# WildBitangent/GMU-Path-Tracer

Measured on AMD Instinct MI355X. Metric: Mpaths/s @1920x1080x64spp, 260k-tri scene, higher is better.
Workload: dtype f32; 1 GPU; config3: 259372-tri seeded sphere room (185137 nodes), 1920x1080, 64 spp steady state, UE4+glass+NEE, unbounded depth; prewarm_steps=2010, tiling=row bands x1, parallelism=tile1

## Files before the change

gmu-path-tracer_amd/build.py:

```python
import os
import subprocess
import sys

HERE = os.path.dirname(os.path.abspath(__file__))
LIB = os.path.join(HERE, "libgmupt.so")

DEVICE_SOURCES = ["csrc/pt_kernels.hip", "csrc/pt_traverse.hip", "csrc/pt_traverse_wide.hip", "csrc/pt_traverse_variants.hip", "csrc/pt_aov.hip", "csrc/pt_denoise.hip", "csrc/pt_temporal.hip", "csrc/pt_refit.hip", "csrc/pt_motion.hip", "csrc/pt_lbvh.hip", "csrc/gmupt_capi.hip"]
HOST_SOURCES = ["csrc/pt_travtables.cpp", "csrc/pt_lbvh.cpp", "host/sbvh_builder.cpp", "host/Camera.cpp", "host/TextureLoader.cpp", "host/AvirResize.cpp"]
HEADERS = ["csrc/pt_traverse_common.hpp", "csrc/pt_shading.hpp", "csrc/pt_denoise.hpp", "csrc/pt_temporal.hpp", "csrc/pt_refit.hpp", "csrc/pt_travtables.hpp", "csrc/pt_motion.hpp", "csrc/pt_lbvh.hpp", "csrc/pt_traverse_deferred.hpp", "csrc/pt_kernel_util.hpp", "host/MeshData.hpp", "host/BVHWrapper.hpp", "csrc/pt_device.hpp", "csrc/detmath.hpp", "host/sbvh_builder.hpp", "host/Camera.hpp", "host/TextureLoader.hpp", "host/png_reader.hpp", "host/Constants.hpp", "../include/gmupt.h"]

FLAGS = [
    "--offload-arch=gfx950", "-O3", "-std=c++17", "-fPIC", "-shared",
    "-ffp-contract=off", "-fhip-fp32-correctly-rounded-divide-sqrt", "-fno-gpu-flush-denormals-to-zero",
    "-fno-fast-math", "-Wall", "-Wno-unused-function",
]


TEST_BUILDS = {"variants": ["-DGMUPT_VARIANTS"], "scan1": ["-DGMUPT_SCAN_GROUP=1"],
               "wides8": ["-DGMUPT_WIDE_STACK=8", "-DGMUPT_WIDE_TOP=64", "-DGMUPT_WIDE_PARK=4"]}
EXPERIMENT_BUILDS = {"wxcd": ["-DGMUPT_WIDE_XCD_EXPERIMENT=1"], "wsg0": ["-DGMUPT_WIDE_SIGNED=0"], "mrg0": ["-DGMUPT_MATERIAL_REGROUP=0"], "wq0": ["-DGMUPT_WIDE_QUADPK=0"], "wqt0": ["-DGMUPT_WIDE_QUADTRI=0"], "dnb0": ["-DGMUPT_DN_BATCH=0"]}


def lib_path(name=None):
    return LIB if not name else os.path.join(HERE, "libgmupt_%s.so" % name)


def needs_build(name=None):
    lib = lib_path(name)
    if not os.path.exists(lib):
        return True
    t = os.path.getmtime(lib)
    deps = DEVICE_SOURCES + HOST_SOURCES + HEADERS + ["build.py"]
    return any(os.path.getmtime(os.path.join(HERE, d)) > t for d in deps if os.path.exists(os.path.join(HERE, d)))


def build(force=False, verbose=False, name=None):
    lib = lib_path(name)
    if not force and not needs_build(name):
        return lib
    hipcc = os.environ.get("HIPCC", "/opt/rocm/bin/hipcc")
    extra = os.environ.get("GMUPT_EXTRA_FLAGS", "").split() + ({**TEST_BUILDS, **EXPERIMENT_BUILDS}[name] if name else [])
    cmd = [hipcc] + FLAGS + extra + ["-x", "hip"] + [os.path.join(HERE, s) for s in DEVICE_SOURCES + HOST_SOURCES] + ["-o", lib]
    if verbose:
        print(" ".join(cmd), file=sys.stderr)
    subprocess.run(cmd, check=True, cwd=HERE)
    return lib


def build_all(force=False, verbose=False):
    from concurrent.futures import ThreadPoolExecutor
    names = [None] + sorted(TEST_BUILDS)
    with ThreadPoolExecutor(len(names)) as ex:
        return list(ex.map(lambda n: build(force=force, verbose=verbose, name=n), names))


if __name__ == "__main__":
    if "--experiments" in sys.argv:
        from concurrent.futures import ThreadPoolExecutor
        with ThreadPoolExecutor(4) as ex:
            print("\n".join(ex.map(lambda n: build(force=True, name=n), sorted(EXPERIMENT_BUILDS))))
    elif "--all" in sys.argv:
        print("\n".join(build_all(force="--force" in sys.argv, verbose=True)))
    else:
        print(build(force="--force" in sys.argv, verbose=True))
```

gmu-path-tracer_amd/capi.py:

```python
import ctypes as C
import os

import numpy as np

from . import build as _build

MAX_LIGHTS = 128
PATHCOUNT = 1 << 21
REF_GRID_THREADS = 34 * 8 * 256
STATE_BYTES = 248

(BUFFER_BVH_NODES, BUFFER_TRIANGLES, BUFFER_VERTICES, BUFFER_LIGHTS, BUFFER_TRI_PROPS, BUFFER_MATERIALS, BUFFER_TEXTURE_ARRAY) = range(7)
STAGE_SHADE, STAGE_EXTEND, STAGE_SHADOW, STAGE_RAYCASTS = range(4)
MATERIAL_UE4, MATERIAL_GLASS = 0, 1

bvh_node_dtype = np.dtype([("min", "<f4", 3), ("pad0", "<f4"), ("max", "<f4", 3), ("pad1", "<f4"),
                           ("left", "<i4"), ("right", "<i4"), ("isLeaf", "<i4"), ("pad2", "<f4")])
triangle_dtype = np.dtype([("v", "<i4", 3), ("materialID", "<u4")])
tri_props_dtype = np.dtype([("normal", "<f4", 3), ("pad0", "<f4"), ("uv", "<f4", 2), ("materialID", "<u4"), ("pad1", "<f4")])
light_dtype = np.dtype([("position", "<f4", 3), ("falloff", "<f4"), ("emission", "<f4", 3), ("radius", "<f4")])
material_dtype = np.dtype([("color", "<f4", 4), ("metallic", "<f4"), ("roughness", "<f4"), ("refractIndex", "<f4"),
                           ("transmittance", "<f4"), ("textureIndices", "<i4", 3), ("materialType", "<u4")])
assert bvh_node_dtype.itemsize == 48 and triangle_dtype.itemsize == 16 and tri_props_dtype.itemsize == 32
assert light_dtype.itemsize == 32 and material_dtype.itemsize == 48
# ... 42 lines not shown
                ("min_leaf_size", C.c_int32), ("max_leaf_size", C.c_int32), ("node_cost", C.c_float), ("tri_cost", C.c_float)]


ERR_INVALID_ARGUMENT, ERR_HIP, ERR_OUT_OF_MEMORY, ERR_NOT_BOUND, ERR_UNSUPPORTED, ERR_IO, ERR_CAST_FAULT = -1, -2, -3, -4, -5, -6, -7
MAX_TRACE_BATCH = 1 << 26


class Ray(C.Structure):
    _fields_ = [("origin", C.c_float * 3), ("tmax", C.c_float), ("direction", C.c_float * 3), ("pad", C.c_uint32)]


class Hit(C.Structure):
    _fields_ = [("t", C.c_float), ("u", C.c_float), ("v", C.c_float), ("triangle", C.c_int32), ("light", C.c_uint32),
                ("material", C.c_uint32), ("pad", C.c_uint32 * 2)]


class TraceInfo(C.Structure):
    _fields_ = [("flags", C.c_uint32), ("pad_", C.c_uint32), ("redo_rays", C.c_uint64), ("ms", C.c_double)]


class Aov(C.Structure):
    _fields_ = [("albedo", C.c_float * 3), ("depth", C.c_float), ("normal", C.c_float * 3), ("roughness", C.c_float),
                ("position", C.c_float * 3), ("metallic", C.c_float), ("triangle", C.c_int32), ("material", C.c_uint32),
                ("light", C.c_uint32), ("coverage", C.c_uint32)]


AOV_MAX_SAMPLES = 8
AOV_CHUNK_RAYS = 1 << 21
assert C.sizeof(Ray) == 32 and C.sizeof(Hit) == 32 and C.sizeof(TraceInfo) == 24 and C.sizeof(Aov) == 64
ray_dtype = np.dtype([("origin", "<f4", 3), ("tmax", "<f4"), ("direction", "<f4", 3), ("pad", "<u4")])
hit_dtype = np.dtype([("t", "<f4"), ("u", "<f4"), ("v", "<f4"), ("triangle", "<i4"), ("light", "<u4"), ("material", "<u4"), ("pad", "<u4", 2)])
aov_dtype = np.dtype([("albedo", "<f4", 3), ("depth", "<f4"), ("normal", "<f4", 3), ("roughness", "<f4"), ("position", "<f4", 3),
                      ("metallic", "<f4"), ("triangle", "<i4"), ("material", "<u4"), ("light", "<u4"), ("coverage", "<u4")])
assert ray_dtype.itemsize == 32 and hit_dtype.itemsize == 32 and aov_dtype.itemsize == 64


class DenoiseParams(C.Structure):
    _fields_ = [("passes", C.c_uint32), ("sigma_color", C.c_float), ("sigma_normal", C.c_float), ("sigma_plane", C.c_float),
                ("sigma_albedo", C.c_float)]


DENOISE_MAX_PASSES = 5
assert C.sizeof(DenoiseParams) == 20


class TemporalParams(C.Structure):
    _fields_ = [("spatial", DenoiseParams), ("history_cap", C.c_float), ("min_normal_cos", C.c_float), ("plane_dist", C.c_float)]


TEMPORAL_MAX_CAP = 65536.0
assert C.sizeof(TemporalParams) == 32
history_dtype = np.dtype([("color", "<f4", 3), ("count", "<f4"), ("normal", "<f4", 3), ("material", "<u4"), ("position", "<f4", 3),
                          ("valid", "<u4")])
assert history_dtype.itemsize == 48
motion_dtype = np.dtype([("prev_position", "<f4", 3), ("flags", "<u4")])
assert motion_dtype.itemsize == 16


class RefitInfo(C.Structure):
    _fields_ = [("rebuilt", C.c_uint32), ("reason", C.c_uint32), ("levels", C.c_uint32), ("opened_nodes", C.c_uint32), ("ms", C.c_double)]


REFIT_FLAT_CHILD, REFIT_VARIANTS_BUILD = 1, 2
assert C.sizeof(RefitInfo) == 24


class LbvhParams(C.Structure):
    _fields_ = [("max_leaf_size", C.c_uint32)]


class LbvhInfo(C.Structure):
    _fields_ = [("num_nodes", C.c_uint32), ("num_leaves", C.c_uint32), ("depth", C.c_uint32), ("num_tris", C.c_uint32),
                ("root_min", C.c_float * 3), ("root_max", C.c_float * 3), ("ms", C.c_double)]

    def as_dict(self):
        return {"num_nodes": int(self.num_nodes), "num_leaves": int(self.num_leaves), "depth": int(self.depth), "num_tris": int(self.num_tris),
                "root_min": np.array(self.root_min[:], np.float32), "root_max": np.array(self.root_max[:], np.float32), "ms": float(self.ms)}


assert C.sizeof(LbvhInfo) == 48


class GmuptError(RuntimeError):
    def __init__(self, msg, code=0):
        super().__init__(msg)
        self.code = code


_P = C.c_void_p
SYMBOLS = {
    "gmupt_device_create": (C.c_int, [C.c_int, C.POINTER(_P)]),
    "gmupt_device_destroy": (None, [_P]),
    "gmupt_last_error": (C.c_char_p, []),
    "gmupt_device_count": (C.c_int, []),
    "gmupt_buffer_create": (C.c_int, [_P, C.c_int, _P, C.c_size_t, C.POINTER(_P)]),
    "gmupt_buffer_update": (C.c_int, [_P, _P, C.c_size_t]),
    "gmupt_buffer_read": (C.c_int, [_P, _P, C.c_size_t]),
    "gmupt_buffer_destroy": (None, [_P]),
    "gmupt_buffer_size": (C.c_size_t, [_P]),
    "gmupt_texture_array_create": (C.c_int, [_P, _P, C.c_uint32, C.c_uint32, C.POINTER(_P)]),
    "gmupt_image_decode_png": (C.c_int, [_P, C.c_size_t, C.POINTER(C.c_uint32), C.POINTER(C.c_uint32), C.POINTER(_P)]),
    "gmupt_image_free": (None, [_P]),
    "gmupt_image_resize_square": (C.c_int, [_P, C.c_uint32, C.c_uint32, _P]),
    "gmupt_texture_common_size": (C.c_uint32, [C.POINTER(C.c_size_t), C.c_uint32]),
    "gmupt_renderer_create": (C.c_int, [_P, C.POINTER(RendererDesc), C.POINTER(_P)]),
    "gmupt_renderer_destroy": (None, [_P]),
    "gmupt_renderer_bind_scene": (C.c_int, [_P] * 7),
    "gmupt_renderer_bind_textures": (C.c_int, [_P, _P, _P, _P]),
    "gmupt_set_camera": (C.c_int, [_P, C.POINTER(CameraBuffer)]),
    "gmupt_iterate": (C.c_int, [_P]),
    "gmupt_resize": (C.c_int, [_P, C.c_uint32, C.c_uint32]),
    "gmupt_read_framebuffer": (C.c_int, [_P, _P, C.c_size_t]),
    "gmupt_copy_framebuffer_to_device": (C.c_int, [_P, _P, C.c_size_t]),
    "gmupt_get_counters": (C.c_int, [_P, C.POINTER(C.c_uint32 * 8)]),
    "gmupt_synchronize": (C.c_int, [_P]),
    "gmupt_get_stats": (C.c_int, [_P, C.POINTER(Stats)]),
    "gmupt_reset_stats": (C.c_int, [_P]),
    "gmupt_enable_timing": (C.c_int, [_P, C.c_int]),
    "gmupt_render_budget": (C.c_int, [_P, _P, C.c_uint32, C.POINTER(C.c_uint32)]),
    "gmupt_trace_rays": (C.c_int, [_P, _P, C.c_uint32, _P, _P, C.c_uint32, _P, C.c_uint32, C.POINTER(TraceInfo)]),
    "gmupt_camera_pick_ray": (C.c_int, [C.POINTER(CameraBuffer), C.c_float, C.c_float, C.POINTER(Ray)]),
    "gmupt_pick": (C.c_int, [_P, C.c_float, C.c_float, C.c_uint32, C.POINTER(Ray), C.POINTER(Hit)]),
    "gmupt_render_aovs": (C.c_int, [_P, C.c_uint32, _P, C.c_size_t, C.POINTER(TraceInfo)]),
    "gmupt_aov_ray": (C.c_int, [C.POINTER(CameraBuffer), C.c_uint32, C.c_uint32, C.c_uint32, C.c_uint32, C.POINTER(Ray)]),
    "gmupt_denoise_default_params": (None, [C.POINTER(DenoiseParams)]),
    "gmupt_denoise_image": (C.c_int, [_P, _P, _P, C.c_uint32, C.c_uint32, C.POINTER(DenoiseParams), _P, C.c_size_t, C.POINTER(C.c_float)]),
    "gmupt_render_denoised": (C.c_int, [_P, C.c_uint32, C.POINTER(DenoiseParams), _P, C.c_size_t, C.POINTER(TraceInfo)]),
    "gmupt_denoise_host": (C.c_int, [_P, _P, C.c_uint32, C.c_uint32, C.POINTER(DenoiseParams), _P, C.c_size_t, C.c_uint32]),
    "gmupt_temporal_default_params": (None, [C.POINTER(TemporalParams)]),
    "gmupt_temporal_create": (C.c_int, [_P, C.POINTER(_P)]),
    "gmupt_temporal_destroy": (None, [_P]),
    "gmupt_temporal_reset": (C.c_int, [_P]),
    "gmupt_temporal_denoise_image": (C.c_int, [_P, _P, _P, C.POINTER(CameraBuffer), C.c_uint32, C.c_uint32, C.c_uint32, C.c_uint32, C.c_int,
                                               C.POINTER(TemporalParams), _P, C.c_size_t, C.POINTER(C.c_float)]),
    "gmupt_render_denoised_temporal": (C.c_int, [_P, _P, C.c_uint32, C.POINTER(TemporalParams), _P, C.c_size_t, C.POINTER(TraceInfo)]),
    "gmupt_temporal_integrate_host": (C.c_int, [_P, _P, C.c_uint32, C.c_uint32, _P, C.POINTER(CameraBuffer), C.c_uint32, C.c_uint32,
                                                C.c_uint32, C.c_uint32, C.POINTER(TemporalParams), _P, _P, C.c_uint32]),
    "gmupt_bvh_refit_host": (C.c_int, [_P, C.c_uint32, _P, C.c_uint32, _P, C.c_uint32, C.c_uint32]),
    "gmupt_renderer_refit": (C.c_int, [_P, C.POINTER(RefitInfo)]),
    "gmupt_render_aovs_motion": (C.c_int, [_P, C.c_uint32, _P, C.c_uint32, _P, C.c_size_t, _P, C.c_size_t, C.POINTER(TraceInfo)]),
    "gmupt_motion_host": (C.c_int, [_P, _P, C.c_size_t, _P, C.c_uint32, _P, _P, C.c_uint32, _P]),
    "gmupt_temporal_integrate_motion_host": (C.c_int, [_P, _P, _P, C.c_uint32, C.c_uint32, _P, C.POINTER(CameraBuffer), C.c_uint32, C.c_uint32,
                                                       C.c_uint32, C.c_uint32, C.POINTER(TemporalParams), _P, _P, C.c_uint32]),
    "gmupt_temporal_denoise_image_motion": (C.c_int, [_P, _P, _P, _P, C.POINTER(CameraBuffer), C.c_uint32, C.c_uint32, C.c_uint32, C.c_uint32, C.c_int,
                                                      C.POINTER(TemporalParams), _P, C.c_size_t, C.POINTER(C.c_float)]),
    "gmupt_render_denoised_temporal_motion": (C.c_int, [_P, _P, C.c_uint32, C.POINTER(TemporalParams), _P, C.c_size_t, C.POINTER(TraceInfo)]),
    "gmupt_lbvh_default_params": (None, [C.POINTER(LbvhParams)]),
    "gmupt_lbvh_build_host": (C.c_int, [_P, C.c_uint32, _P, C.c_uint32, _P, C.POINTER(LbvhParams), _P, _P, _P, C.POINTER(LbvhInfo)]),
    "gmupt_lbvh_create": (C.c_int, [_P, C.POINTER(_P)]),
    "gmupt_lbvh_destroy": (None, [_P]),
    "gmupt_lbvh_build": (C.c_int, [_P, _P, _P, C.c_uint32, _P, C.POINTER(LbvhParams), C.POINTER(_P), C.POINTER(_P), _P, C.POINTER(LbvhInfo)]),
    "gmupt_debug_read_path_state": (C.c_int, [_P, _P, C.c_size_t]),
    "gmupt_debug_write_path_state": (C.c_int, [_P, _P, C.c_size_t]),
    "gmupt_debug_read_queues": (C.c_int, [_P, _P, C.c_size_t]),
    "gmupt_debug_write_queues": (C.c_int, [_P, _P, C.c_size_t]),
    "gmupt_debug_write_counters": (C.c_int, [_P, C.POINTER(C.c_uint32 * 8)]),
    "gmupt_debug_write_framebuffer": (C.c_int, [_P, _P, C.c_size_t]),
    "gmupt_debug_run_stage": (C.c_int, [_P, C.c_int]),
    "gmupt_debug_detmath": (C.c_int, [_P, C.c_int, _P, _P, _P, C.c_uint32]),
    "gmupt_debug_travtables_build": (C.c_int, [_P, C.c_uint32, _P, C.c_uint32, _P, C.c_uint32, C.c_int, C.c_int, C.c_int, C.POINTER(_P)]),
    "gmupt_debug_travtables_data": (_P, [_P, C.c_int, C.POINTER(C.c_size_t)]),
    "gmupt_debug_travtables_destroy": (None, [_P]),
    "gmupt_debug_wide_tables_addressable": (C.c_int, [C.c_uint32, C.c_uint32, C.c_uint32]),
    "gmupt_sbvh_default_params": (None, [C.POINTER(SbvhParams)]),
    "gmupt_sbvh_build": (C.c_int, [_P, C.c_uint32, _P, C.c_uint32, C.POINTER(SbvhParams), C.POINTER(_P)]),
    "gmupt_sbvh_num_nodes": (C.c_uint32, [_P]),
    "gmupt_sbvh_num_references": (C.c_uint32, [_P]),
    "gmupt_sbvh_sah": (C.c_float, [_P]),
    "gmupt_sbvh_depth": (C.c_uint32, [_P]),
    "gmupt_sbvh_flatten": (C.c_int, [_P, _P, _P, _P, _P]),
    "gmupt_sbvh_destroy": (None, [_P]),
    "gmupt_camera_create": (C.c_int, [C.c_uint32, C.c_uint32, C.POINTER(_P)]),
    "gmupt_camera_destroy": (None, [_P]),
    "gmupt_camera_update_resolution": (None, [_P, C.c_uint32, C.c_uint32]),
    "gmupt_camera_set_pose": (None, [_P, C.c_float, C.c_float, C.c_float, C.c_float, C.c_float]),
    "gmupt_camera_update": (None, [_P, C.c_float]),
    "gmupt_camera_set_input": (None, [_P, C.c_float, C.c_float, C.c_uint32]),
    "gmupt_camera_reset_accumulation": (None, [_P]),
    "gmupt_camera_get_buffer": (C.POINTER(CameraBuffer), [_P]),
    "gmupt_version": (C.c_char_p, []),
}

_lib = None
_libs = {}
_devices_created = 0


def _load(path):
    if path not in _libs:
        handle = C.CDLL(path)
        for name, (res, args) in SYMBOLS.items():
            fn = getattr(handle, name)
            fn.restype = res
            fn.argtypes = args
        _libs[path] = handle
    return _libs[path]


def lib():
    global _lib
    if _lib is None:
        path = os.environ.get("GMUPT_LIB") or _build.LIB
        if not os.environ.get("GMUPT_LIB") and (not os.path.exists(path) or (os.path.exists("/opt/rocm/bin/hipcc") and _build.needs_build())):
            path = _build.build()
        _lib = _load(path)
    return _lib


class use_build:

    def __init__(self, name):
        self.name = name

    def __enter__(self):
        global _lib
        path = _build.lib_path(self.name)
        if not os.path.exists(path) or (os.path.exists("/opt/rocm/bin/hipcc") and _build.needs_build(self.name)):
            if _devices_created:
                raise GmuptError("test build %r is missing or older than its sources and this process already uses the GPU: run __graft_entry__.build() first" % self.name)
            path = _build.build(name=self.name)
        self.saved = lib()
        _lib = _load(path)
        return _lib

    def __exit__(self, *exc):
        global _lib
        _lib = self.saved
        return False


def _check(rc):
    if rc != 0:
        raise GmuptError("gmupt error %d: %s" % (rc, lib().gmupt_last_error().decode(errors="replace")), rc)


def _ptr(a):
    return a.ctypes.data_as(C.c_void_p)


class Device:
    def __init__(self, index=0):
        global _devices_created
        self.h = _P()
        _check(lib().gmupt_device_create(index, C.byref(self.h)))
        _devices_created += 1
        self.index = index

    def close(self):
        if self.h:
            lib().gmupt_device_destroy(self.h)
            self.h = _P()

    def detmath(self, fn, x, y=None):
        x = np.ascontiguousarray(x, dtype=np.float32)
        y = np.zeros_like(x) if y is None else np.ascontiguousarray(y, dtype=np.float32)
        out = np.empty_like(x)
        _check(lib().gmupt_debug_detmath(self.h, fn, _ptr(x), _ptr(y), _ptr(out), x.size))
        return out


class Buffer:
    def __init__(self, dev, kind, array):
        array = np.ascontiguousarray(array)
        self.h = _P()
        self.dev = dev
        _check(lib().gmupt_buffer_create(dev.h, kind, _ptr(array), array.nbytes, C.byref(self.h)))

    @classmethod
    def wrap(cls, dev, handle):
        self = cls.__new__(cls)
        self.h, self.dev = handle, dev
        return self

    def update(self, array):
        array = np.ascontiguousarray(array)
        _check(lib().gmupt_buffer_update(self.h, _ptr(array), array.nbytes))

    def read(self, dtype=np.uint8):
        dtype = np.dtype(dtype)
        nbytes = int(lib().gmupt_buffer_size(self.h))
        out = np.empty(nbytes // dtype.itemsize, dtype=dtype)
        _check(lib().gmupt_buffer_read(self.h, _ptr(out), out.nbytes))
        return out

    def close(self):
        if self.h:
            lib().gmupt_buffer_destroy(self.h)
            self.h = _P()


class TextureArray:

    def __init__(self, dev, array):
        array = np.ascontiguousarray(array, dtype=np.uint8)
        assert array.ndim == 4 and array.shape[1] == array.shape[2] and array.shape[3] == 4
        self.h = _P()
        _check(lib().gmupt_texture_array_create(dev.h, _ptr(array), array.shape[1], array.shape[0], C.byref(self.h)))

    def close(self):
        if self.h:
            lib().gmupt_buffer_destroy(self.h)
            self.h = _P()


def decode_png(data):
    w, h, mem = C.c_uint32(), C.c_uint32(), _P()
    buf = (C.c_uint8 * len(data)).from_buffer_copy(bytes(data))
    _check(lib().gmupt_image_decode_png(buf, len(data), C.byref(w), C.byref(h), C.byref(mem)))
    try:
        out = np.ctypeslib.as_array(C.cast(mem, C.POINTER(C.c_uint8)), shape=(h.value, w.value, 4)).copy()
    finally:
        lib().gmupt_image_free(mem)
    return out


def resize_square(rgba, new_size):
    rgba = np.ascontiguousarray(rgba, dtype=np.uint8)
    assert rgba.ndim == 3 and rgba.shape[0] == rgba.shape[1] and rgba.shape[2] == 4
    out = np.empty((new_size, new_size, 4), dtype=np.uint8)
    _check(lib().gmupt_image_resize_square(_ptr(rgba), rgba.shape[0], new_size, _ptr(out)))
    return out


def texture_common_size(layer_bytes):
    arr = (C.c_size_t * len(layer_bytes))(*layer_bytes)
    return int(lib().gmupt_texture_common_size(arr, len(layer_bytes)))


def texture_array_from_png(files):
    layers = [decode_png(f) for f in files]
    for l in layers:
        if l.shape[0] != l.shape[1]:
            raise GmuptError("texture is not square")
    size = texture_common_size([l.size for l in layers])
    return np.stack([l if l.shape[0] == size else resize_square(l, size) for l in layers])


class SceneBuffers:

    def __init__(self, dev, scene):
        self.nodes = Buffer(dev, BUFFER_BVH_NODES, scene["nodes"])
        self.tris = Buffer(dev, BUFFER_TRIANGLES, scene["tris"])
        self.verts = Buffer(dev, BUFFER_VERTICES, scene["verts"])
        self.lights = Buffer(dev, BUFFER_LIGHTS, scene["lights"])
        self.props = Buffer(dev, BUFFER_TRI_PROPS, scene["props"])
        self.materials = Buffer(dev, BUFFER_MATERIALS, scene["materials"])
        self.textures = [TextureArray(dev, scene[k]) if scene.get(k) is not None else None
                         for k in ("tex_diffuse", "tex_metallic_roughness", "tex_normal")]

    def all(self):
        return [self.nodes, self.tris, self.verts, self.lights, self.props, self.materials]

    def close(self):
        for b in self.all():
            b.close()
        for t in self.textures:
            if t is not None:
                t.close()


class Camera:

    def __init__(self, width, height):
        self.h = _P()
        _check(lib().gmupt_camera_create(width, height, C.byref(self.h)))

    def set_pose(self, x, y, z, pitch, yaw):
        lib().gmupt_camera_set_pose(self.h, x, y, z, pitch, yaw)

    def update(self, dt=0.0):
        lib().gmupt_camera_update(self.h, dt)

    def update_resolution(self, width, height):
        lib().gmupt_camera_update_resolution(self.h, width, height)

    def reset_accumulation(self):
        lib().gmupt_camera_reset_accumulation(self.h)

    def set_input(self, mouse_dx=0.0, mouse_dy=0.0, w=False, s=False, a=False, d=False):
        lib().gmupt_camera_set_input(self.h, mouse_dx, mouse_dy, (1 if w else 0) | (2 if s else 0) | (4 if a else 0) | (8 if d else 0))

    @property
    def buffer(self):
        return lib().gmupt_camera_get_buffer(self.h).contents

    def buffer_copy(self):
        out = CameraBuffer()
        C.memmove(C.byref(out), C.byref(self.buffer), C.sizeof(CameraBuffer))
        return out

    def close(self):
        if self.h:
            lib().gmupt_camera_destroy(self.h)
            self.h = _P()


class Renderer:
    def __init__(self, dev, width, height, pool_paths=0, live_paths=0, tile=None, path_budget=0, max_depth=0, collect_stats=False):
        d = RendererDesc(width, height, pool_paths, live_paths, 0, 0, 0, path_budget, max_depth, 1 if collect_stats else 0)
        if tile is not None:
            d.tile_enabled, d.tile_x0, d.tile_y0 = 1, tile[0], tile[1]
        self.desc = d
        self.dev = dev
        self.h = _P()
        _check(lib().gmupt_renderer_create(dev.h, C.byref(d), C.byref(self.h)))
        self.width, self.height = width, height
        self.pool = pool_paths or PATHCOUNT
        self._scene = None
        self._temporals = []

    def bind_scene(self, sb):
        self._scene = sb
        _check(lib().gmupt_renderer_bind_scene(self.h, *[b.h for b in sb.all()]))
        _check(lib().gmupt_renderer_bind_textures(self.h, *[(t.h if t is not None else None) for t in sb.textures]))

    def refit(self):
        info = RefitInfo()
        _check(lib().gmupt_renderer_refit(self.h, C.byref(info)))
        return {k: getattr(info, k) for k, _ in RefitInfo._fields_}

    def set_camera(self, cam_buffer):
        _check(lib().gmupt_set_camera(self.h, C.byref(cam_buffer)))

    def iterate(self):
        _check(lib().gmupt_iterate(self.h))

    def run_stage(self, stage):
        _check(lib().gmupt_debug_run_stage(self.h, stage))

    def synchronize(self):
        _check(lib().gmupt_synchronize(self.h))

    def resize(self, w, h):
        _check(lib().gmupt_resize(self.h, w, h))
        self.width, self.height = w, h

    def framebuffer(self):
        out = np.empty((self.height, self.width, 4), dtype=np.float32)
        _check(lib().gmupt_read_framebuffer(self.h, _ptr(out), out.nbytes))
        return out

    def copy_framebuffer_to_device(self, device_ptr, nbytes):
        _check(lib().gmupt_copy_framebuffer_to_device(self.h, C.c_void_p(device_ptr), nbytes))

    def counters(self):
        out = (C.c_uint32 * 8)()
        _check(lib().gmupt_get_counters(self.h, C.byref(out)))
        return np.array(list(out), dtype=np.uint32)

    def stats(self, check=True):
        s = Stats()
        rc = lib().gmupt_get_stats(self.h, C.byref(s))
        if rc != ERR_CAST_FAULT or check:
            _check(rc)
        return s

    def reset_stats(self):
        _check(lib().gmupt_reset_stats(self.h))

    def enable_timing(self, mode=1):
        _check(lib().gmupt_enable_timing(self.h, int(mode)))

    def render_budget(self, camera, max_iterations=1 << 20):
        it = C.c_uint32(0)
        _check(lib().gmupt_render_budget(self.h, camera.h, max_iterations, C.byref(it)))
        return it.value

    def trace(self, closest=None, any=None, light_count=0, info=None):
        import torch
        dev = torch.device("cuda", getattr(self.dev, "index", 0))
        as_numpy = isinstance(closest, np.ndarray) or isinstance(any, np.ndarray)

        def stage(a):
            if a is None:
                return torch.empty((0, 8), dtype=torch.float32, device=dev)
            t = torch.from_numpy(np.ascontiguousarray(a, dtype=np.float32).reshape(-1, 8)).to(dev) if isinstance(a, np.ndarray) else a
            if t.dtype != torch.float32 or t.dim() != 2 or t.shape[1] != 8 or not t.is_cuda:
                raise GmuptError("trace: rays must be (N, 8) float32 on the GPU (or numpy)", ERR_INVALID_ARGUMENT)
            return t.contiguous()

        c, a = stage(closest), stage(any)
        hits = torch.empty((c.shape[0], 8), dtype=torch.float32, device=dev)
        occ = torch.empty((a.shape[0],), dtype=torch.int32, device=dev)
        torch.cuda.current_stream(dev).synchronize()
        ti = info if info is not None else TraceInfo()
        ptr = lambda t: C.c_void_p(t.data_ptr()) if t.numel() else None
        _check(lib().gmupt_trace_rays(self.h, ptr(c), c.shape[0], ptr(hits), ptr(a), a.shape[0], ptr(occ), int(light_count), C.byref(ti)))
        self.last_trace = ti
        if as_numpy:
            return hits.cpu().numpy(), occ.cpu().numpy().view(np.uint32)
        return hits, occ

    def pick(self, px, py, light_count=0):
        ray, hit = Ray(), Hit()
        _check(lib().gmupt_pick(self.h, float(px), float(py), int(light_count), C.byref(ray), C.byref(hit)))
        return ray, hit

    def aovs(self, samples=1, info=None):
        import torch
        dev = torch.device("cuda", getattr(self.dev, "index", 0))
        out = torch.empty((self.height, self.width, 16), dtype=torch.float32, device=dev)
        torch.cuda.current_stream(dev).synchronize()
        ti = info if info is not None else TraceInfo()
        _check(lib().gmupt_render_aovs(self.h, int(samples), C.c_void_p(out.data_ptr()), out.numel() * 4, C.byref(ti)))
        self.last_aovs = ti
        return out

    def aovs_motion(self, prev_verts, samples=1, info=None):
        import torch
        dev = torch.device("cuda", getattr(self.dev, "index", 0))
        if not hasattr(prev_verts, "is_cuda") or not prev_verts.is_cuda or prev_verts.dtype != torch.float32 or prev_verts.numel() % 3:
            raise GmuptError("aovs_motion: prev_verts must be a float32 tensor of 3 floats per vertex on the GPU", ERR_INVALID_ARGUMENT)
        if prev_verts.device.index != dev.index:
            raise GmuptError("aovs_motion: prev_verts lives on %s, the renderer on %s" % (prev_verts.device, dev), ERR_INVALID_ARGUMENT)
        pv = prev_verts.contiguous()
        out = torch.empty((self.height, self.width, 16), dtype=torch.float32, device=dev)
        mv = torch.empty((self.height, self.width, 4), dtype=torch.float32, device=dev)
        torch.cuda.current_stream(dev).synchronize()
        ti = info if info is not None else TraceInfo()
        _check(lib().gmupt_render_aovs_motion(self.h, int(samples), C.c_void_p(pv.data_ptr()), pv.numel() // 3, C.c_void_p(out.data_ptr()),
                                              out.numel() * 4, C.c_void_p(mv.data_ptr()), mv.numel() * 4, C.byref(ti)))
        self.last_aovs = ti
        return out, mv

    def denoise(self, aov_samples=1, info=None, **params):
        import torch
        dev = torch.device("cuda", getattr(self.dev, "index", 0))
        out = torch.empty((self.height, self.width, 4), dtype=torch.float32, device=dev)
        dp = denoise_params(**params)
        torch.cuda.current_stream(dev).synchronize()
        ti = info if info is not None else TraceInfo()
        _check(lib().gmupt_render_denoised(self.h, int(aov_samples), C.byref(dp), C.c_void_p(out.data_ptr()), out.numel() * 4, C.byref(ti)))
        self.last_denoise = ti
        return out

    def denoise_temporal(self, handle, aov_samples=1, info=None, **params):
        import torch
        dev = torch.device("cuda", getattr(self.dev, "index", 0))
        out = torch.empty((self.height, self.width, 4), dtype=torch.float32, device=dev)
        tp = temporal_params(**params)
        torch.cuda.current_stream(dev).synchronize()
        ti = info if info is not None else TraceInfo()
        _check(lib().gmupt_render_denoised_temporal(self.h, handle.h, int(aov_samples), C.byref(tp), C.c_void_p(out.data_ptr()), out.numel() * 4,
                                                    C.byref(ti)))
        self.last_denoise = ti
        return out

    def denoise_temporal_motion(self, handle, aov_samples=1, info=None, **params):
        import torch
        dev = torch.device("cuda", getattr(self.dev, "index", 0))
        out = torch.empty((self.height, self.width, 4), dtype=torch.float32, device=dev)
        tp = temporal_params(**params)
        torch.cuda.current_stream(dev).synchronize()
        ti = info if info is not None else TraceInfo()
        _check(lib().gmupt_render_denoised_temporal_motion(self.h, handle.h, int(aov_samples), C.byref(tp), C.c_void_p(out.data_ptr()),
                                                           out.numel() * 4, C.byref(ti)))
        self.last_denoise = ti
        return out

    def read_path_state(self):
        out = np.empty(self.pool * STATE_BYTES, dtype=np.uint8)
        _check(lib().gmupt_debug_read_path_state(self.h, _ptr(out), out.nbytes))
        return out

    def write_path_state(self, raw):
        raw = np.ascontiguousarray(raw, dtype=np.uint8)
        _check(lib().gmupt_debug_write_path_state(self.h, _ptr(raw), raw.nbytes))

    def read_queues(self):
        out = np.empty(self.pool * 5, dtype=np.uint32)
        _check(lib().gmupt_debug_read_queues(self.h, _ptr(out), out.nbytes))
        return out.reshape(5, self.pool)

    def write_queues(self, q):
        q = np.ascontiguousarray(q, dtype=np.uint32)
        _check(lib().gmupt_debug_write_queues(self.h, _ptr(q), q.nbytes))

    def write_counters(self, qc):
        arr = (C.c_uint32 * 8)(*[int(v) for v in qc])
        _check(lib().gmupt_debug_write_counters(self.h, C.byref(arr)))

    def write_framebuffer(self, fb):
        fb = np.ascontiguousarray(fb, dtype=np.float32)
        _check(lib().gmupt_debug_write_framebuffer(self.h, _ptr(fb), fb.nbytes))

    def close(self):
        if self.h:
            for t in self._temporals:
                t.close()
            lib().gmupt_renderer_destroy(self.h)
            self.h = _P()


class Temporal:

    def __init__(self, renderer):
        self.renderer = renderer
        self.h = _P()
        _check(lib().gmupt_temporal_create(renderer.h, C.byref(self.h)))
        renderer._temporals.append(self)

    def reset(self):
        _check(lib().gmupt_temporal_reset(self.h))

    def close(self):
        if self.h:
            lib().gmupt_temporal_destroy(self.h)
            self.h = _P()


def camera_pick_ray(cam_buffer, px, py):
    ray = Ray()
    _check(lib().gmupt_camera_pick_ray(C.byref(cam_buffer), float(px), float(py), C.byref(ray)))
    return ray


def hit_fields(hits):
    h = hits.cpu().numpy() if hasattr(hits, "cpu") else np.asarray(hits)
    rec = np.ascontiguousarray(h, dtype=np.float32).reshape(-1, 8).view(hit_dtype)[:, 0]
    return {k: rec[k].copy() for k in ("t", "u", "v", "triangle", "light", "material")}


def aov_ray(cam_buffer, x, y, samples, k):
    ray = Ray()
    _check(lib().gmupt_aov_ray(C.byref(cam_buffer), int(x), int(y), int(samples), int(k), C.byref(ray)))
    return ray


def aov_rays(cam_buffer, xs, ys, samples):
    R = 1 if samples == 1 else samples * samples + 1
    out = np.empty((len(xs), R, 8), np.float32)
    for i, (x, y) in enumerate(zip(xs, ys)):
        for k in range(R):
            out[i, k] = np.frombuffer(bytes(aov_ray(cam_buffer, x, y, samples, k)), np.float32)
    return out


def aov_fields(aovs):
    a = aovs.cpu().numpy() if hasattr(aovs, "cpu") else np.asarray(aovs)
    a = np.ascontiguousarray(a, dtype=np.float32)
    rec = a.reshape(-1, 16).view(aov_dtype)[:, 0]
    shape = a.shape[:-1]
    return {k: rec[k].reshape(shape + rec[k].shape[1:]).copy() for k in aov_dtype.names}


def denoise_params(**params):
    dp = DenoiseParams()
    lib().gmupt_denoise_default_params(C.byref(dp))
    for k, v in params.items():
        if k not in ("passes", "sigma_color", "sigma_normal", "sigma_plane", "sigma_albedo"):
            raise TypeError("unknown denoiser parameter %r" % k)
        setattr(dp, k, v)
    return dp


def denoise_image(renderer, beauty, aov, ms=None, **params):
    import torch
    if beauty.dim() != 3 or beauty.shape[2] != 4 or aov.dim() != 3 or aov.shape[2] != 16 or tuple(aov.shape[:2]) != tuple(beauty.shape[:2]):
        raise GmuptError("denoise_image: beauty must be (H, W, 4) and aov (H, W, 16)", ERR_INVALID_ARGUMENT)
    if beauty.dtype != torch.float32 or aov.dtype != torch.float32 or not beauty.is_cuda or not aov.is_cuda:
        raise GmuptError("denoise_image: float32 tensors on the GPU", ERR_INVALID_ARGUMENT)
    beauty, aov = beauty.contiguous(), aov.contiguous()
    H, W = beauty.shape[0], beauty.shape[1]
    out = torch.empty_like(beauty)
    dp = denoise_params(**params)
    torch.cuda.current_stream(beauty.device).synchronize()
    t = C.c_float(0.0)
    _check(lib().gmupt_denoise_image(renderer.h, C.c_void_p(beauty.data_ptr()), C.c_void_p(aov.data_ptr()), W, H, C.byref(dp),
                                     C.c_void_p(out.data_ptr()), out.numel() * 4, C.byref(t)))
    if ms is not None:
        ms.append(t.value)
    return out


def denoise_host(beauty, aov, threads=16, **params):
    b = beauty.cpu().numpy() if hasattr(beauty, "cpu") else np.asarray(beauty)
    a = aov.cpu().numpy() if hasattr(aov, "cpu") else np.asarray(aov)
    b = np.ascontiguousarray(b, dtype=np.float32)
    if a.dtype == aov_dtype:
        a = a.view(np.float32).reshape(a.shape + (16,))
    a = np.ascontiguousarray(a, dtype=np.float32)
    if b.ndim != 3 or b.shape[2] != 4 or a.shape != b.shape[:2] + (16,):
        raise GmuptError("denoise_host: beauty must be (H, W, 4) and aov (H, W, 16)", ERR_INVALID_ARGUMENT)
    out = np.empty_like(b)
    dp = denoise_params(**params)
    _check(lib().gmupt_denoise_host(_ptr(b), _ptr(a), b.shape[1], b.shape[0], C.byref(dp), _ptr(out), out.nbytes, int(threads)))
    return out


TEMPORAL_FIELDS = ("history_cap", "min_normal_cos", "plane_dist")


def temporal_params(**params):
    tp = TemporalParams()
    lib().gmupt_temporal_default_params(C.byref(tp))
    for k, v in params.items():
        if k in TEMPORAL_FIELDS:
            setattr(tp, k, v)
        elif k in ("passes", "sigma_color", "sigma_normal", "sigma_plane", "sigma_albedo"):
            setattr(tp.spatial, k, v)
        else:
            raise TypeError("unknown temporal denoiser parameter %r" % k)
    return tp


def temporal_denoise_image(handle, beauty, aov, cam_buffer, new_accumulation, origin=(0, 0), ms=None, motion=None, **params):
    import torch
    if beauty.dim() != 3 or beauty.shape[2] != 4 or aov.dim() != 3 or aov.shape[2] != 16 or tuple(aov.shape[:2]) != tuple(beauty.shape[:2]):
        raise GmuptError("temporal_denoise_image: beauty must be (H, W, 4) and aov (H, W, 16)", ERR_INVALID_ARGUMENT)
    if beauty.dtype != torch.float32 or aov.dtype != torch.float32 or not beauty.is_cuda or not aov.is_cuda:
        raise GmuptError("temporal_denoise_image: float32 tensors on the GPU", ERR_INVALID_ARGUMENT)
    beauty, aov = beauty.contiguous(), aov.contiguous()
    H, W = beauty.shape[0], beauty.shape[1]
    out = torch.empty_like(beauty)
    tp = temporal_params(**params)
    if motion is not None:
        if motion.dtype != torch.float32 or not motion.is_cuda or tuple(motion.shape) != (H, W, 4) or motion.device != beauty.device:
            raise GmuptError("temporal_denoise_image: motion must be an (H, W, 4) float32 tensor on the GPU of beauty", ERR_INVALID_ARGUMENT)
        hdev = getattr(handle.renderer.dev, "index", 0)
        if beauty.device.index != hdev or aov.device != beauty.device:
# ... 247 lines not shown
```

gmu-path-tracer_amd/csrc/gmupt_capi.hip:

```cpp
#include "pt_device.hpp"
#include "detmath.hpp"
#include "pt_shading.hpp"
#include "pt_denoise.hpp"
#include "pt_temporal.hpp"
#include "pt_refit.hpp"
#include "pt_motion.hpp"
#include "pt_travtables.hpp"
#include "pt_lbvh.hpp"
#include "../host/sbvh_builder.hpp"
#include "../host/Camera.hpp"
#include "../host/TextureLoader.hpp"
#include "../host/png_reader.hpp"

#include <hip/hip_runtime.h>
#include <algorithm>
#include <array>
#include <cmath>
#include <cstdarg>
#include <cstdio>
#include <cstdlib>
#include <cstring>
#include <limits>
#include <string>
#include <unordered_map>
// ... 167 lines not shown
extern "C" uint32_t gmupt_texture_common_size(const size_t* layer_bytes, uint32_t layers)
{
    if (!layer_bytes || layers == 0) return 0;
    return gmupt::commonDimension(std::vector<size_t>(layer_bytes, layer_bytes + layers));
}

extern "C" int gmupt_texture_array_create(gmupt_device* dev, const uint8_t* rgba8, uint32_t size, uint32_t layers, gmupt_buffer** out)
{
    if (!dev || !out || !rgba8) return fail(GMUPT_ERR_INVALID_ARGUMENT, "gmupt_texture_array_create: null argument");
    if (size == 0 || layers == 0 || size > 16384) return fail(GMUPT_ERR_INVALID_ARGUMENT, "gmupt_texture_array_create: %u layers of %ux%u", layers, size, size);
    int rc = gmupt_buffer_create(dev, GMUPT_BUFFER_TEXTURE_ARRAY, rgba8, (size_t)size * size * layers * 4, out);
    if (rc == GMUPT_OK) { (*out)->texSize = size; (*out)->texLayers = layers; }
    return rc;
}

extern "C" int gmupt_buffer_update(gmupt_buffer* buf, const void* data, size_t bytes)
{
    if (!buf || (!data && bytes)) return fail(GMUPT_ERR_INVALID_ARGUMENT, "gmupt_buffer_update: null argument");
    if (bytes > buf->bytes) return fail(GMUPT_ERR_INVALID_ARGUMENT, "gmupt_buffer_update: %zu bytes into a %zu-byte buffer", bytes, buf->bytes);
    HIP_TRY(hipSetDevice(buf->dev->id));
    HIP_TRY(hipDeviceSynchronize());
    HIP_TRY(hipMemcpy(buf->dptr, data, bytes, hipMemcpyHostToDevice));
    return GMUPT_OK;
}

extern "C" int gmupt_buffer_read(const gmupt_buffer* buf, void* dst, size_t bytes)
{
    if (!buf || (!dst && bytes)) return fail(GMUPT_ERR_INVALID_ARGUMENT, "gmupt_buffer_read: null argument");
    if (bytes > buf->bytes) return fail(GMUPT_ERR_INVALID_ARGUMENT, "gmupt_buffer_read: %zu bytes from a %zu-byte buffer", bytes, buf->bytes);
    HIP_TRY(hipSetDevice(buf->dev->id));
    HIP_TRY(hipDeviceSynchronize());
    HIP_TRY(hipMemcpy(dst, buf->dptr, bytes, hipMemcpyDeviceToHost));
    return GMUPT_OK;
}

extern "C" void gmupt_buffer_destroy(gmupt_buffer* buf)
{
    if (!buf) return;
    (void)hipSetDevice(buf->dev->id);
    (void)hipFree(buf->dptr);
    delete buf;
}

extern "C" size_t gmupt_buffer_size(const gmupt_buffer* buf) { return buf ? buf->bytes : 0; }

struct StageEvents { hipEvent_t e[5]; bool extOnly = false; };

struct gmupt_renderer {
    gmupt_device* dev = nullptr;
    gmupt_renderer_desc desc{};
    hipStream_t stream = nullptr;
    RenderParams p{};
    bool sceneBound = false, cameraSet = false;
    uint64_t iterations = 0;
    uint32_t travBlocks = 0;
    int timing = 0;
    std::vector<StageEvents> evPool; size_t evUsed = 0;
    double msStage[4] = { 0, 0, 0, 0 }; uint64_t timedIters = 0;
    std::vector<void*> allocs;
    void* travNodes = nullptr; void* travTris = nullptr; void* travRecs = nullptr; void* travWide = nullptr; void* travPairs = nullptr; void* travPairRef = nullptr;
    int travMode = 70;
    uint32_t castFlags = 0;
    uint32_t* queryCounters = nullptr; DevStats* queryStats = nullptr; void* pickBuf = nullptr;
    hipEvent_t queryEv[2] = { nullptr, nullptr };
    gmupt_ray* aovRays = nullptr; gmupt_hit* aovHits = nullptr;
    void* dnScratch = nullptr; size_t dnScratchBytes = 0;
    void* dnInput = nullptr; size_t dnInputBytes = 0;
    hipEvent_t dnEv[2] = { nullptr, nullptr };
    uint64_t accumGeneration = 0;
    uint64_t bindingId = 0, geomGeneration = 0;
    const gmupt_buffer* boundNodes = nullptr; const gmupt_buffer* boundTris = nullptr; const gmupt_buffer* boundVerts = nullptr;
    size_t boundElems[3] = { 0, 0, 0 };
    std::vector<uint32_t> rfLevelNodes, rfLevelOff, rfNodeMap, rfWideMap, rfOpened;
    void* rfDev = nullptr;
    hipEvent_t rfEv[2] = { nullptr, nullptr };
};

static std::array<void**, 6> trav_tables(gmupt_renderer* r) { return { &r->travNodes, &r->travTris, &r->travRecs, &r->travWide, &r->travPairs, &r->travPairRef }; }

static int dev_alloc(gmupt_renderer* r, void** ptr, size_t bytes, int fill)
{
    *ptr = nullptr;
    HIP_TRY(hipMalloc(ptr, bytes ? bytes : 16));
    r->allocs.push_back(*ptr);
    HIP_TRY(hipMemsetAsync(*ptr, fill, bytes ? bytes : 16, r->stream));
    return GMUPT_OK;
}

static int alloc_framebuffer(gmupt_renderer* r, uint32_t w, uint32_t h)
{
    void* fb = nullptr; void* head = nullptr;
    const size_t npix = (size_t)w * h;
    HIP_TRY(hipMalloc(&fb, npix * 16 + 16));
    HIP_TRY(hipMalloc(&head, npix * 4 + 16));
    HIP_TRY(hipMemsetAsync(fb, 0, npix * 16 + 16, r->stream));
    HIP_TRY(hipMemsetAsync(head, 0xFF, npix * 4 + 16, r->stream));
    r->p.fb = (float4*)fb; r->p.listHead = (uint32_t*)head; r->p.fbW = w; r->p.fbH = h;
    return GMUPT_OK;
}

extern "C" void gmupt_renderer_destroy(gmupt_renderer* r)
{
    if (!r) return;
    (void)hipSetDevice(r->dev->id);
    if (r->stream) (void)hipStreamSynchronize(r->stream);
    for (auto& se : r->evPool) for (auto& e : se.e) (void)hipEventDestroy(e);
    for (hipEvent_t e : r->queryEv) if (e) (void)hipEventDestroy(e);
    for (hipEvent_t e : r->dnEv) if (e) (void)hipEventDestroy(e);
    for (hipEvent_t e : r->rfEv) if (e) (void)hipEventDestroy(e);
    if (r->rfDev) (void)hipFree(r->rfDev);
    for (void* a : r->allocs) (void)hipFree(a);
    if (r->dnScratch) (void)hipFree(r->dnScratch);
    if (r->dnInput) (void)hipFree(r->dnInput);
    if (r->p.fb) (void)hipFree(r->p.fb);
    if (r->p.listHead) (void)hipFree(r->p.listHead);
    for (void** t : trav_tables(r)) if (*t) (void)hipFree(*t);
    if (r->stream) (void)hipStreamDestroy(r->stream);
    delete r;
}

static int parse_traversal_mode(const char* tv)
{
    constexpr int kDefault = 70;
    if (!tv || !*tv) return kDefault;
    if (std::strcmp(tv, "whilewhile") == 0) return 0;
    if (std::strcmp(tv, "ref") == 0) return 1;
    if (std::strcmp(tv, "static") == 0) return 2;
    if (std::strncmp(tv, "ifif", 4) == 0) return 3 + std::atoi(tv + 4);
    if (std::strcmp(tv, "coop") == 0) return 20;
    if (std::strcmp(tv, "top") == 0) return 30;
    if (std::strncmp(tv, "def", 3) == 0) return 40 + std::atoi(tv + 3);
    if (std::strncmp(tv, "pipe", 4) == 0) return 50 + std::atoi(tv + 4);
    if (std::strncmp(tv, "cast", 4) == 0) return 60 + std::atoi(tv + 4);
    if (std::strcmp(tv, "wide") == 0) return 70;
    return kDefault;
}

extern "C" int gmupt_renderer_create(gmupt_device* dev, const gmupt_renderer_desc* desc, gmupt_renderer** out)
{
    if (!dev || !desc || !out) return fail(GMUPT_ERR_INVALID_ARGUMENT, "gmupt_renderer_create: null argument");
    *out = nullptr;
    if (desc->width == 0 || desc->height == 0) return fail(GMUPT_ERR_INVALID_ARGUMENT, "gmupt_renderer_create: empty accumulation target %ux%u", desc->width, desc->height);
    gmupt_renderer* r = new (std::nothrow) gmupt_renderer();
    if (!r) return fail(GMUPT_ERR_OUT_OF_MEMORY, "gmupt_renderer_create: out of host memory");
    r->dev = dev; r->desc = *desc;
    r->travMode = parse_traversal_mode(std::getenv("GMUPT_TRAVERSAL"));
    if (!traversal_mode_available(r->travMode)) {
        delete r;
        return fail(GMUPT_ERR_UNSUPPORTED, "gmupt_renderer_create: GMUPT_TRAVERSAL=%s is not part of this build (wide, cast0 and def0 are; the other rungs need -DGMUPT_VARIANTS)", std::getenv("GMUPT_TRAVERSAL"));
    }
    if (r->desc.pool_paths == 0) r->desc.pool_paths = GMUPT_PATHCOUNT;
    if (r->desc.live_paths == 0 || r->desc.live_paths > r->desc.pool_paths) r->desc.live_paths = r->desc.pool_paths;
    const uint32_t P = r->desc.pool_paths, L = r->desc.live_paths;
    if ((uint64_t)P * F_COUNT * 4ull > (200ull << 30)) { delete r; return fail(GMUPT_ERR_INVALID_ARGUMENT, "gmupt_renderer_create: pool of %u paths is too large", P); }

    hipError_t e = hipSetDevice(dev->id);
    if (e == hipSuccess) e = hipStreamCreateWithFlags(&r->stream, hipStreamNonBlocking);
    if (e != hipSuccess) { delete r; return fail(GMUPT_ERR_HIP, "gmupt_renderer_create: %s", hipGetErrorString(e)); }

    RenderParams& p = r->p;
    p.P = P; p.L = L;
    p.nBlocks = (L + kBlock - 1) / kBlock;
    p.tileEnabled = desc->tile_enabled; p.tileX0 = desc->tile_x0; p.tileY0 = desc->tile_y0;
    p.budget = desc->path_budget; p.maxDepth = desc->max_depth;
    const uint32_t tb = traversal_block_threads();
    r->travBlocks = (L + tb - 1) / tb;
    p.ovfStride = r->travBlocks * tb;
    if (p.ovfStride < deferred_block_threads()) p.ovfStride = deferred_block_threads();
    { const char* rw = std::getenv("GMUPT_RAYS_PER_WAVE"); p.raysPerWave = rw ? (uint32_t)std::atoi(rw) : 128u; if (p.raysPerWave < 64) p.raysPerWave = 64; if (r->travMode >= 60 && p.raysPerWave > 128) p.raysPerWave = 128;  }
    { const char* wpc = std::getenv("GMUPT_WAVES_PER_CU"); const uint32_t w = wpc ? (uint32_t)std::atoi(wpc) : 16u; const uint32_t db = deferred_block_threads(); p.travGridBlocks = (uint32_t)dev->prop.multiProcessorCount * ((w * 64 + db - 1) / db); if (p.travGridBlocks * db > p.ovfStride) p.travGridBlocks = p.ovfStride / db; if (p.travGridBlocks == 0) p.travGridBlocks = 1; }
    { const char* ep = std::getenv("GMUPT_EXTEND_PRUNE"); p.extendPrune = ep ? (uint32_t)std::atoi(ep) : 0u; }
    { const char* sp = std::getenv("GMUPT_SHADOW_PRUNE"); p.shadowPrune = sp ? (uint32_t)std::atoi(sp) : 0u; }
    { const char* ws = std::getenv("GMUPT_WIDE_STEPS"); p.tuneWideSteps = ws ? (uint32_t)std::atoi(ws) : 0u; }
    { const char* xb = std::getenv("GMUPT_XCD_BINS"); p.xcdBins = xb ? (uint32_t)std::atoi(xb) : 0u; }
    { const char* lc = std::getenv("GMUPT_CAST_LOOP_CAP"); p.castLoopCap = lc ? (uint32_t)std::atoi(lc) : (1u << 20); if (p.castLoopCap == 0) p.castLoopCap = 1u << 20; }
    { const char* e1 = std::getenv("GMUPT_REFILL"); p.tuneRefill = e1 ? (uint32_t)std::atoi(e1) : 20u; const char* e2 = std::getenv("GMUPT_TRI_THRESH"); p.tuneTriThresh = e2 ? (uint32_t)std::atoi(e2) : ((r->travMode == 60 || r->travMode == 63 || r->travMode == 70) ? 24u : 32u); }

    int rc = GMUPT_OK;
    { const char* pad = std::getenv("GMUPT_STATE_PAD"); p.PS = P + (pad ? (uint32_t)std::atoi(pad) & ~63u : 1088u); }
    if (rc == GMUPT_OK) rc = dev_alloc(r, (void**)&p.state, (size_t)F_COUNT * p.PS * 4, 0);
    if (rc == GMUPT_OK) rc = dev_alloc(r, (void**)&p.cls, (size_t)P, CLS_ENDED);
    if (rc == GMUPT_OK) rc = dev_alloc(r, (void**)&p.listNext, (size_t)P * 4, 0xFF);
    if (rc == GMUPT_OK) rc = dev_alloc(r, (void**)&p.sample, (size_t)P * 12, 0);
    if (rc == GMUPT_OK) rc = dev_alloc(r, (void**)&p.blockCounts, (size_t)p.nBlocks * 4 * kNumCounts, 0);
    p.nGroups = (p.nBlocks + kScanGroup - 1) / kScanGroup; p.groupParity = 0;
    if (rc == GMUPT_OK) rc = dev_alloc(r, (void**)&p.groupTotals, (size_t)2 * kNumCounts * p.nGroups * 4, 0);
    if (rc == GMUPT_OK) rc = dev_alloc(r, (void**)&p.queues, (size_t)P * 20, 0);
    if (rc == GMUPT_OK) rc = dev_alloc(r, (void**)&p.qc, 32, 0);
    if (rc == GMUPT_OK) rc = dev_alloc(r, (void**)&p.stats, sizeof(DevStats), 0);
    if (rc == GMUPT_OK) rc = dev_alloc(r, (void**)&p.travCounters, 128, 0);
    if (rc == GMUPT_OK) rc = dev_alloc(r, (void**)&p.ovfStack, (size_t)p.ovfStride * traversal_overflow_entries() * 4, 0);
    if (rc == GMUPT_OK) rc = alloc_framebuffer(r, desc->width, desc->height);
    if (rc == GMUPT_OK) {
        DevStats init{}; init.activePaths = L;
        e = hipMemcpyAsync(p.stats, &init, sizeof(init), hipMemcpyHostToDevice, r->stream);
        if (e == hipSuccess) e = hipStreamSynchronize(r->stream);
        if (e != hipSuccess) rc = fail(GMUPT_ERR_HIP, "gmupt_renderer_create: %s", hipGetErrorString(e));
    }
    if (rc != GMUPT_OK) { std::string keep = g_lastError; gmupt_renderer_destroy(r); g_lastError = keep; return rc; }
    *out = r;
    return GMUPT_OK;
}

static TravOptions trav_options(bool wantWide)
{
    const char* order = std::getenv("GMUPT_TOP_ORDER");
    const char* pairing = std::getenv("GMUPT_NODE_PAIRING");
    TravOptions o;
    o.wantWide = wantWide; o.topOrderBfs = order && std::strcmp(order, "bfs") == 0; o.nodePairing = !(pairing && std::atoi(pairing) == 0);
    o.topCapacity = traversal_top_capacity; o.wideTopCapacity = traversal_wide_top_capacity();
    return o;
}

static int build_traversal_copy(gmupt_renderer* r, const gmupt_buffer* nodesB, const gmupt_buffer* trisB, const gmupt_buffer* vertsB)
{
    HIP_TRY(hipSetDevice(r->dev->id));
    HIP_TRY(hipStreamSynchronize(r->stream));
    const size_t N = nodesB->elems, R = trisB->elems, V = vertsB->elems;
    std::vector<gmupt_bvh_node> nodes(N);
    std::vector<gmupt_triangle> tris(R ? R : 1);
    std::vector<float> verts(V ? V * 3 : 3);
    HIP_TRY(hipMemcpy(nodes.data(), nodesB->dptr, N * sizeof(gmupt_bvh_node), hipMemcpyDeviceToHost));
    if (R) HIP_TRY(hipMemcpy(tris.data(), trisB->dptr, R * sizeof(gmupt_triangle), hipMemcpyDeviceToHost));
    if (V) HIP_TRY(hipMemcpy(verts.data(), vertsB->dptr, V * 12, hipMemcpyDeviceToHost));

    TravTables tt;
    const std::string err = build_trav_tables(nodes.data(), N, tris.data(), R, verts.data(), V, trav_options(r->travMode == 70), tt);
    if (!err.empty()) return fail(GMUPT_ERR_INVALID_ARGUMENT, "%s", err.c_str());

    const bool haveWide = !tt.wide.empty();
    const void* recs = nullptr; size_t recBytes = 0;
#ifdef GMUPT_VARIANTS
    recs = tt.recs.data(); recBytes = tt.recs.size() * sizeof(Rec64);
#endif
    const struct { const void* data; size_t bytes; } up[6] = {
        { tt.nodes.data(), tt.nodes.size() * sizeof(Node64) }, { tt.tris.data(), tt.tris.size() * sizeof(Tri48) }, { recs, recBytes },
        { tt.wide.data(), tt.wide.size() * sizeof(WNode) }, { tt.pairs.data(), haveWide ? tt.pairs.size() * sizeof(TriPair) : 0 },
        { tt.pairRef.data(), haveWide ? tt.pairRef.size() * 4 : 0 } };
    const std::array<void**, 6> dst = trav_tables(r);
    for (int k = 0; k < 6; k++) {
        if (*dst[k]) { HIP_TRY(hipFree(*dst[k])); *dst[k] = nullptr; }
        if (!up[k].bytes) continue;
        HIP_TRY(hipMalloc(dst[k], up[k].bytes));
        HIP_TRY(hipMemcpy(*dst[k], up[k].data, up[k].bytes, hipMemcpyHostToDevice));
    }
    TravScene& t = r->p.trav;
    t.recs = (const Rec64*)r->travRecs; t.nodes = (const Node64*)r->travNodes; t.tris = (const Tri48*)r->travTris;
    t.wnodes = (const WNode*)r->travWide; t.pairs = (const TriPair*)r->travPairs; t.pairRef = (const uint32_t*)r->travPairRef;
    t.triBase = tt.s.triBase; t.rootDesc = tt.s.rootDesc; t.topCount = tt.s.topCount; t.topCountDeep = tt.s.topCountDeep; t.maxDepth = tt.s.maxDepth;
    for (int k = 0; k < 3; k++) { t.rootMin[k] = tt.s.rootMin[k]; t.rootMax[k] = tt.s.rootMax[k]; }
    t.wideCount = tt.s.wideCount; t.wideTopCount = tt.s.wideTopCount; t.wideStackBound = tt.s.wideStackBound; t.wideRootDesc = 0; t.numPairs = tt.s.numPairs;

    if (r->rfDev) { HIP_TRY(hipFree(r->rfDev)); r->rfDev = nullptr; }
    r->rfLevelNodes.swap(tt.levelNodes); r->rfLevelOff.swap(tt.levelOff); r->rfNodeMap.swap(tt.nodeMap); r->rfWideMap.swap(tt.wideMap); r->rfOpened.swap(tt.opened);
    r->boundNodes = nodesB; r->boundTris = trisB; r->boundVerts = vertsB;
    r->boundElems[0] = N; r->boundElems[1] = R; r->boundElems[2] = V;
    return GMUPT_OK;
}

static_assert(sizeof(gmupt_refit_info) == 24 && offsetof(gmupt_refit_info, ms) == 16, "gmupt_refit_info layout");

extern "C" int gmupt_renderer_refit(gmupt_renderer* r, gmupt_refit_info* info)
{
    if (!r) return fail(GMUPT_ERR_INVALID_ARGUMENT, "gmupt_renderer_refit: null renderer");
    if (info) *info = gmupt_refit_info{};
    if (!r->sceneBound) return fail(GMUPT_ERR_NOT_BOUND, "gmupt_renderer_refit: no scene bound");
    if (r->boundNodes->elems != r->boundElems[0] || r->boundTris->elems != r->boundElems[1] || r->boundVerts->elems != r->boundElems[2])
        return fail(GMUPT_ERR_INVALID_ARGUMENT, "gmupt_renderer_refit: the bound buffers hold (%zu, %zu, %zu) nodes / triangle records / vertices, at bind time (%zu, %zu, %zu)",
                    r->boundNodes->elems, r->boundTris->elems, r->boundVerts->elems, r->boundElems[0], r->boundElems[1], r->boundElems[2]);
    HIP_TRY(hipSetDevice(r->dev->id));
    HIP_TRY(hipStreamSynchronize(r->stream));
    const std::vector<uint32_t>* maps[4] = { &r->rfLevelNodes, &r->rfNodeMap, &r->rfWideMap, &r->rfOpened };
    size_t off[4], words = 16;
    for (int k = 0; k < 4; k++) { off[k] = words; words += (maps[k]->size() + 3) & ~(size_t)3; }
    if (!r->rfDev) {
        HIP_TRY(hipMalloc(&r->rfDev, words * 4));
        for (int k = 0; k < 4; k++)
            if (!maps[k]->empty()) HIP_TRY(hipMemcpy((uint32_t*)r->rfDev + off[k], maps[k]->data(), maps[k]->size() * 4, hipMemcpyHostToDevice));
    }
    for (hipEvent_t& e : r->rfEv) if (!e) HIP_TRY(hipEventCreate(&e));
    uint32_t* dev = (uint32_t*)r->rfDev;
    const TravScene& t = r->p.trav;
    RfArgs a{};
    a.nodes = (DNode*)r->boundNodes->dptr; a.tris = (const gmupt_triangle*)r->boundTris->dptr; a.verts = (const float*)r->boundVerts->dptr;
    a.numNodes = (uint32_t)r->boundElems[0]; a.numTris = (uint32_t)r->boundElems[1]; a.numVerts = (uint32_t)r->boundElems[2];
    a.levelNodes = dev + off[0];
    a.ttris = (Tri48*)r->travTris; a.pairs = (TriPair*)r->travPairs; a.pairRef = t.pairRef; a.numPairs = t.numPairs;
    a.tnodes = (Node64*)r->travNodes; a.nodeMap = dev + off[1]; a.numPacked = (uint32_t)r->rfNodeMap.size();
    a.wnodes = (WNode*)r->travWide; a.wideMap = dev + off[2]; a.wideCount = r->travWide ? t.wideCount : 0u;
    a.opened = dev + off[3]; a.numOpened = r->travWide ? (uint32_t)r->rfOpened.size() : 0u;
    a.flags = dev;

    uint32_t back[16] = { 0 };
    HIP_TRY(hipMemsetAsync(dev, 0, 64, r->stream));
    launch_refit_check(a, r->stream);
    HIP_TRY(hipGetLastError());
    HIP_TRY(hipMemcpyAsync(back, dev, 4, hipMemcpyDeviceToHost, r->stream));
    HIP_TRY(hipStreamSynchronize(r->stream));
    if (back[0] & kRfFlagBadIndex) return fail(GMUPT_ERR_INVALID_ARGUMENT, "gmupt_renderer_refit: a triangle record references a vertex outside the vertex buffer (the triangle records changed since bind)");
    if (back[0] & kRfFlagNonFinite) return fail(GMUPT_ERR_INVALID_ARGUMENT, "gmupt_renderer_refit: a vertex used by a triangle record is not finite; nothing was written");

    uint32_t reason = 0;
#ifdef GMUPT_VARIANTS
    reason = GMUPT_REFIT_VARIANTS_BUILD;
#endif
    HIP_TRY(hipEventRecord(r->rfEv[0], r->stream));
    const uint32_t levels = launch_refit_boxes(a, r->rfLevelOff, r->stream);
    if (!reason) launch_refit_tables(a, r->stream);
    HIP_TRY(hipGetLastError());
    HIP_TRY(hipMemcpyAsync(dev + 4, a.nodes, 32, hipMemcpyDeviceToDevice, r->stream));
    HIP_TRY(hipEventRecord(r->rfEv[1], r->stream));
    HIP_TRY(hipMemcpyAsync(back, dev, 64, hipMemcpyDeviceToHost, r->stream));
    HIP_TRY(hipStreamSynchronize(r->stream));
    float ms = 0.0f;
    HIP_TRY(hipEventElapsedTime(&ms, r->rfEv[0], r->rfEv[1]));
    if (back[1]) reason |= GMUPT_REFIT_FLAT_CHILD;
    const uint32_t openedNodes = a.numOpened;
    if (reason) {
        int rc = build_traversal_copy(r, r->boundNodes, r->boundTris, r->boundVerts);
        if (rc != GMUPT_OK) return rc;
    } else {
        for (int k = 0; k < 3; k++) { std::memcpy(&r->p.trav.rootMin[k], &back[4 + k], 4); std::memcpy(&r->p.trav.rootMax[k], &back[8 + k], 4); }
    }
    r->geomGeneration++;
    if (info) { info->rebuilt = reason ? 1u : 0u; info->reason = reason; info->levels = levels; info->opened_nodes = openedNodes; info->ms = (double)ms; }
    return GMUPT_OK;
}

extern "C" int gmupt_bvh_refit_host(gmupt_bvh_node* nodes, uint32_t num_nodes, const gmupt_triangle* tris, uint32_t num_tris,
                                    const float* verts, uint32_t num_verts, uint32_t threads)
{
    if (!nodes || num_nodes == 0 || (!tris && num_tris) || (!verts && num_verts)) return fail(GMUPT_ERR_INVALID_ARGUMENT, "gmupt_bvh_refit_host: null or empty array");
    const std::string err = validate_tree("gmupt_bvh_refit_host", nodes, num_nodes, tris, num_tris, num_verts, 0);
// ... 783 lines not shown
    if (rc != GMUPT_OK) return rc;
    HIP_TRY(hipSetDevice(r->dev->id));
    const bool fold = !t->seen || t->generation != r->accumGeneration;
    TpSlot& fz = fold ? t->last : t->frozen;
    TpSlot& nw = fold ? t->frozen : t->last;
    const uint32_t nv = r->p.scene.numVerts;
    const auto inPose = [&](const TpSlot& sl) { return sl.hasPose && sl.binding == r->bindingId && sl.numVerts == nv; };
    const bool moved = poses && fz.present && inPose(fz) && fz.geomGeneration != r->geomGeneration;
    const size_t npix = (size_t)W * H;
    rc = grow_scratch(r, &r->dnInput, &r->dnInputBytes, npix * (sizeof(gmupt_aov) + 16 + (moved ? sizeof(gmupt_motion) : 0)));
    if (rc != GMUPT_OK) return rc;
    gmupt_aov* aov = static_cast<gmupt_aov*>(r->dnInput);
    float* beauty = reinterpret_cast<float*>(static_cast<char*>(r->dnInput) + npix * sizeof(gmupt_aov));
    gmupt_motion* motion = moved ? reinterpret_cast<gmupt_motion*>(static_cast<char*>(r->dnInput) + npix * (sizeof(gmupt_aov) + 16)) : nullptr;
    gmupt_trace_info ai;
    if (moved) rc = gmupt_render_aovs_motion(r, aov_samples, static_cast<const float*>(fz.verts), nv, aov, npix * sizeof(gmupt_aov), motion, npix * sizeof(gmupt_motion), &ai);
    else rc = gmupt_render_aovs(r, aov_samples, aov, npix * sizeof(gmupt_aov), &ai);
    if (info) *info = ai;
    if (rc != GMUPT_OK) return rc;
    rc = gmupt_copy_framebuffer_to_device(r, beauty, npix * 16);
    if (rc != GMUPT_OK) return rc;
    if (poses && !(inPose(nw) && nw.geomGeneration == r->geomGeneration)) {
        nw.hasPose = false;
        rc = grow_scratch(r, &nw.verts, &nw.vertsBytes, (size_t)nv * 12);
        if (rc != GMUPT_OK) return rc;
        HIP_TRY(hipMemcpyAsync(nw.verts, r->p.scene.verts, (size_t)nv * 12, hipMemcpyDeviceToDevice, r->stream));
    }
    const uint32_t x0 = r->p.tileEnabled ? r->p.tileX0 : 0u, y0 = r->p.tileEnabled ? r->p.tileY0 : 0u;
    float ms = 0.0f;
    rc = temporal_denoise(fn, t, beauty, aov, motion, &r->p.cam, x0, y0, W, H, fold ? 1 : 0, p, out_rgba, bytes, &ms);
    if (info) info->ms = ai.ms + ms;
    if (rc != GMUPT_OK) return rc;
    t->seen = true; t->generation = r->accumGeneration;
    if (poses) { t->last.hasPose = true; t->last.binding = r->bindingId; t->last.geomGeneration = r->geomGeneration; t->last.numVerts = nv; }
    return GMUPT_OK;
}

static int temporal_integrate_host(const char* fn, const float* beauty_rgba, const gmupt_aov* aov, const gmupt_motion* motion, uint32_t width, uint32_t height,
                                   const gmupt_history* prev, const gmupt_camera_buffer* prev_cam, uint32_t prev_x0, uint32_t prev_y0,
                                   uint32_t prev_width, uint32_t prev_height, const gmupt_temporal_params* p,
                                   float* out_rgba, gmupt_history* out_history, uint32_t threads)
{
    if (!beauty_rgba || !aov || !out_rgba || !out_history) return fail(GMUPT_ERR_INVALID_ARGUMENT, "%s: null beauty, aov or output", fn);
    if (width == 0 || height == 0 || width > 65535 || height > 65535 || (uint64_t)width * height > (1ull << 28))
        return fail(GMUPT_ERR_INVALID_ARGUMENT, "%s: image of %ux%u (1..65535 each, at most 2^28 pixels)", fn, width, height);
    if (prev) {
        if (!prev_cam) return fail(GMUPT_ERR_INVALID_ARGUMENT, "%s: a previous record set without its camera", fn);
        if (prev_width == 0 || prev_height == 0 || prev_width > 65535 || prev_height > 65535 || (uint64_t)prev_width * prev_height > (1ull << 28) ||
            prev_x0 > 65535 || prev_y0 > 65535)
            return fail(GMUPT_ERR_INVALID_ARGUMENT, "%s: previous rectangle of %ux%u at (%u, %u) (1..65535 each, at most 2^28 pixels)", fn, prev_width, prev_height, prev_x0, prev_y0);
    }
    {
        const size_t n = (size_t)width * height;
        const uintptr_t o[2] = { (uintptr_t)out_rgba, (uintptr_t)out_history }, on[2] = { n * 16, n * sizeof(gmupt_history) };
        const uintptr_t i[5] = { (uintptr_t)beauty_rgba, (uintptr_t)aov, (uintptr_t)prev, (uintptr_t)motion, (uintptr_t)out_history },
                        in[5] = { n * 16, n * sizeof(gmupt_aov), prev ? (size_t)prev_width * prev_height * sizeof(gmupt_history) : 0,
                                  motion ? n * sizeof(gmupt_motion) : 0, n * sizeof(gmupt_history) };
        for (int a = 0; a < 2; a++)
            for (int b = 0; b < (a == 0 ? 5 : 4); b++)
                if (in[b] && o[a] < i[b] + in[b] && i[b] < o[a] + on[a]) return fail(GMUPT_ERR_INVALID_ARGUMENT, "%s: an output overlaps another array", fn);
    }
    gmupt_temporal_params d;
    if (!p) { gmupt_temporal_default_params(&d); p = &d; }
    DnParams dn; TpParams tp;
    int rc = temporal_params(fn, p, dn, tp);
    if (rc != GMUPT_OK) return rc;
    try {
        temporal_host(beauty_rgba, aov, motion, (int)width, (int)height, prev, prev_cam, (int)prev_x0, (int)prev_y0, (int)prev_width, (int)prev_height, tp,
                      out_rgba, out_history, (int)std::min(std::max(threads, 1u), 16u));
    } catch (const std::bad_alloc&) {
        return fail(GMUPT_ERR_OUT_OF_MEMORY, "%s: out of host memory for %ux%u pixels", fn, width, height);
    } catch (const std::exception& e) {
        return fail(GMUPT_ERR_INVALID_ARGUMENT, "%s: %s", fn, e.what());
    }
    return GMUPT_OK;
}

extern "C" int gmupt_temporal_integrate_host(const float* beauty_rgba, const gmupt_aov* aov, uint32_t width, uint32_t height,
                                             const gmupt_history* prev, const gmupt_camera_buffer* prev_cam, uint32_t prev_x0, uint32_t prev_y0,
                                             uint32_t prev_width, uint32_t prev_height, const gmupt_temporal_params* p,
                                             float* out_rgba, gmupt_history* out_history, uint32_t threads)
{
    return temporal_integrate_host("gmupt_temporal_integrate_host", beauty_rgba, aov, nullptr, width, height, prev, prev_cam, prev_x0, prev_y0, prev_width,
                                   prev_height, p, out_rgba, out_history, threads);
}

extern "C" int gmupt_temporal_integrate_motion_host(const float* beauty_rgba, const gmupt_aov* aov, const gmupt_motion* motion, uint32_t width, uint32_t height,
                                                    const gmupt_history* prev, const gmupt_camera_buffer* prev_cam, uint32_t prev_x0, uint32_t prev_y0,
                                                    uint32_t prev_width, uint32_t prev_height, const gmupt_temporal_params* p,
                                                    float* out_rgba, gmupt_history* out_history, uint32_t threads)
{
    return temporal_integrate_host("gmupt_temporal_integrate_motion_host", beauty_rgba, aov, motion, width, height, prev, prev_cam, prev_x0, prev_y0, prev_width,
                                   prev_height, p, out_rgba, out_history, threads);
}

extern "C" int gmupt_motion_host(const gmupt_hit* hits, const gmupt_aov* aov, size_t n, const gmupt_triangle* tris, uint32_t num_tris,
                                 const float* verts_now, const float* verts_prev, uint32_t num_verts, gmupt_motion* out)
{
    const char* fn = "gmupt_motion_host";
    if (n == 0) return GMUPT_OK;
    if (!hits || !aov || !out || !tris || !verts_now || !verts_prev) return fail(GMUPT_ERR_INVALID_ARGUMENT, "%s: null array", fn);
    for (size_t i = 0; i < n; i++) {
        gmupt_hit h;
        std::memcpy(&h, (const char*)hits + i * sizeof(h), sizeof(h));
        if (h.triangle < 0 || h.light > 0u) continue;
        if ((uint32_t)h.triangle >= num_tris) return fail(GMUPT_ERR_INVALID_ARGUMENT, "%s: hit %zu names triangle record %d of %u", fn, i, h.triangle, num_tris);
        gmupt_triangle T;
        std::memcpy(&T, (const char*)tris + (size_t)h.triangle * sizeof(T), sizeof(T));
        for (int k = 0; k < 3; k++)
            if (T.v[k] < 0 || (uint32_t)T.v[k] >= num_verts) return fail(GMUPT_ERR_INVALID_ARGUMENT, "%s: triangle record %d references vertex %d of %u", fn, h.triangle, T.v[k], num_verts);
    }
    motion_host(hits, aov, n, tris, verts_now, verts_prev, out);
    return GMUPT_OK;
}

struct gmupt_camera { Camera cam; gmupt_camera(uint32_t w, uint32_t h) : cam(w, h) {} };

extern "C" int gmupt_render_budget(gmupt_renderer* r, gmupt_camera* cam, uint32_t max_iterations, uint32_t* iters)
{
    if (!r || !cam) return fail(GMUPT_ERR_INVALID_ARGUMENT, "gmupt_render_budget: null argument");
    if (!r->desc.path_budget) return fail(GMUPT_ERR_INVALID_ARGUMENT, "gmupt_render_budget: renderer was created without a path_budget");
    HIP_TRY(hipSetDevice(r->dev->id));
    static_assert(offsetof(DevStats, stackOverflow) == offsetof(DevStats, activePaths) + 4, "the drain check reads both words with one copy");
    uint32_t* hostActive = nullptr;
    HIP_TRY(hipHostMalloc((void**)&hostActive, 8, hipHostMallocDefault));
    hostActive[0] = 1; hostActive[1] = 0;
    uint32_t k = 0;
    int rc = GMUPT_OK;
    constexpr uint32_t kDrainHorizon = 512;
    uint32_t drainStart = 0xFFFFFFFFu;
    for (; k < max_iterations; k++) {
        cam->cam.update(0.0f);
        rc = gmupt_set_camera(r, cam->cam.getBuffer());
        if (rc == GMUPT_OK) rc = gmupt_iterate(r);
        if (rc != GMUPT_OK) break;
        if ((k & 7u) == 7u) {
            hipError_t e = hipMemcpyAsync(hostActive, &r->p.stats->activePaths, 8, hipMemcpyDeviceToHost, r->stream);
            if (e == hipSuccess) e = hipStreamSynchronize(r->stream);
            if (e != hipSuccess) { rc = fail(GMUPT_ERR_HIP, "gmupt_render_budget: %s", hipGetErrorString(e)); break; }
            if (hostActive[1] & 3u) { rc = fail(GMUPT_ERR_CAST_FAULT, "gmupt_render_budget: a ray-cast launch flagged its results as invalid after %u iterations (flags %#x)", k + 1, hostActive[1]); k++; break; }
            if (*hostActive == 0) { k++; break; }
            if (*hostActive < r->p.L && drainStart == 0xFFFFFFFFu) drainStart = k;
            if (drainStart != 0xFFFFFFFFu && k - drainStart >= kDrainHorizon) { k++; break; }
        }
    }
    (void)hipHostFree(hostActive);
    if (rc == GMUPT_OK) { hipError_t e = hipStreamSynchronize(r->stream); if (e != hipSuccess) rc = fail(GMUPT_ERR_HIP, "gmupt_render_budget: %s", hipGetErrorString(e)); }
    if (rc == GMUPT_OK) rc = check_cast_flags(r, "gmupt_render_budget");
    if (iters) *iters = k;
    return rc;
}

namespace {
struct FieldMap { uint32_t refOffset, slotBytes, comps, first; };
const FieldMap kFieldMap[] = {
    { 0, 16, 3, F_RAY_OX }, { 16, 16, 3, F_RAY_DX }, { 32, 16, 3, F_MAT_R }, { 48, 8, 2, F_MAT_METALLIC }, { 56, 16, 3, F_NRM_X },
    { 72, 16, 3, F_SP_X }, { 88, 16, 3, F_BARY_X }, { 104, 4, 1, F_HIT_DIST }, { 108, 16, 4, F_TRI_0 }, { 124, 16, 3, F_SH_OX },
    { 140, 16, 3, F_SH_DX }, { 156, 4, 1, F_LIGHT_IDX }, { 160, 4, 1, F_LIGHT_DIST }, { 164, 4, 1, F_IN_SHADOW }, { 168, 16, 3, F_RAD_R },
    { 184, 16, 3, F_THR_R }, { 200, 16, 3, F_LTHR_R }, { 216, 16, 3, F_DL_R }, { 232, 4, 1, F_PATH_LEN }, { 236, 8, 2, F_SCR_X }, { 244, 4, 1, F_IS_EMITTER },
};
}

extern "C" int gmupt_debug_read_path_state(gmupt_renderer* r, void* dst, size_t bytes)
{
    if (!r || !dst) return fail(GMUPT_ERR_INVALID_ARGUMENT, "gmupt_debug_read_path_state: null argument");
    const size_t P = r->p.P;
    if (bytes < P * GMUPT_STATE_BYTES) return fail(GMUPT_ERR_INVALID_ARGUMENT, "gmupt_debug_read_path_state: %zu bytes given, %zu needed", bytes, P * (size_t)GMUPT_STATE_BYTES);
    HIP_TRY(hipSetDevice(r->dev->id));
    const size_t PS = r->p.PS;
    std::vector<uint32_t> soa((size_t)F_COUNT * PS);
    HIP_TRY(hipMemcpyAsync(soa.data(), r->p.state, soa.size() * 4, hipMemcpyDeviceToHost, r->stream));
    HIP_TRY(hipStreamSynchronize(r->stream));
    std::memset(dst, 0, P * GMUPT_STATE_BYTES);
    uint8_t* out = (uint8_t*)dst;
    for (const FieldMap& f : kFieldMap)
        for (size_t i = 0; i < P; i++) {
            uint32_t* o = (uint32_t*)(out + (size_t)f.refOffset * P + (size_t)f.slotBytes * i);
            for (uint32_t c = 0; c < f.comps; c++) o[c] = soa[(size_t)(f.first + c) * PS + i];
        }
    return GMUPT_OK;
}

extern "C" int gmupt_debug_write_path_state(gmupt_renderer* r, const void* src, size_t bytes)
{
    if (!r || !src) return fail(GMUPT_ERR_INVALID_ARGUMENT, "gmupt_debug_write_path_state: null argument");
    const size_t P = r->p.P;
    if (bytes < P * GMUPT_STATE_BYTES) return fail(GMUPT_ERR_INVALID_ARGUMENT, "gmupt_debug_write_path_state: %zu bytes given, %zu needed", bytes, P * (size_t)GMUPT_STATE_BYTES);
    HIP_TRY(hipSetDevice(r->dev->id));
    const size_t PS = r->p.PS;
    std::vector<uint32_t> soa((size_t)F_COUNT * PS);
    const uint8_t* in = (const uint8_t*)src;
    for (const FieldMap& f : kFieldMap)
        for (size_t i = 0; i < P; i++) {
            const uint32_t* o = (const uint32_t*)(in + (size_t)f.refOffset * P + (size_t)f.slotBytes * i);
            for (uint32_t c = 0; c < f.comps; c++) soa[(size_t)(f.first + c) * PS + i] = o[c];
        }
    HIP_TRY(hipMemcpyAsync(r->p.state, soa.data(), soa.size() * 4, hipMemcpyHostToDevice, r->stream));
    HIP_TRY(hipStreamSynchronize(r->stream));
    return GMUPT_OK;
}

extern "C" int gmupt_debug_read_queues(gmupt_renderer* r, uint32_t* dst, size_t bytes)
{
    if (!r || !dst) return fail(GMUPT_ERR_INVALID_ARGUMENT, "gmupt_debug_read_queues: null argument");
    const size_t need = (size_t)r->p.P * 20;
    if (bytes < need) return fail(GMUPT_ERR_INVALID_ARGUMENT, "gmupt_debug_read_queues: %zu bytes given, %zu needed", bytes, need);
    HIP_TRY(hipSetDevice(r->dev->id));
    HIP_TRY(hipMemcpyAsync(dst, r->p.queues, need, hipMemcpyDeviceToHost, r->stream));
    HIP_TRY(hipStreamSynchronize(r->stream));
    return GMUPT_OK;
}

extern "C" int gmupt_debug_write_queues(gmupt_renderer* r, const uint32_t* src, size_t bytes)
{
    if (!r || !src) return fail(GMUPT_ERR_INVALID_ARGUMENT, "gmupt_debug_write_queues: null argument");
    const size_t need = (size_t)r->p.P * 20;
    if (bytes < need) return fail(GMUPT_ERR_INVALID_ARGUMENT, "gmupt_debug_write_queues: %zu bytes given, %zu needed", bytes, need);
    HIP_TRY(hipSetDevice(r->dev->id));
    HIP_TRY(hipMemcpyAsync(r->p.queues, src, need, hipMemcpyHostToDevice, r->stream));
    HIP_TRY(hipStreamSynchronize(r->stream));
    return GMUPT_OK;
}

extern "C" int gmupt_debug_write_counters(gmupt_renderer* r, const uint32_t in[8])
{
    if (!r || !in) return fail(GMUPT_ERR_INVALID_ARGUMENT, "gmupt_debug_write_counters: null argument");
    HIP_TRY(hipSetDevice(r->dev->id));
    HIP_TRY(hipMemcpyAsync(r->p.qc, in, 32, hipMemcpyHostToDevice, r->stream));
    HIP_TRY(hipStreamSynchronize(r->stream));
    return GMUPT_OK;
}

extern "C" int gmupt_debug_write_framebuffer(gmupt_renderer* r, const float* rgba, size_t bytes)
{
    if (!r || !rgba) return fail(GMUPT_ERR_INVALID_ARGUMENT, "gmupt_debug_write_framebuffer: null argument");
    const size_t need = (size_t)r->p.fbW * r->p.fbH * 16;
    if (bytes < need) return fail(GMUPT_ERR_INVALID_ARGUMENT, "gmupt_debug_write_framebuffer: %zu bytes given, %zu needed", bytes, need);
    HIP_TRY(hipSetDevice(r->dev->id));
    HIP_TRY(hipMemcpyAsync(r->p.fb, rgba, need, hipMemcpyHostToDevice, r->stream));
    HIP_TRY(hipStreamSynchronize(r->stream));
    return GMUPT_OK;
}

extern "C" int gmupt_debug_detmath(gmupt_device* dev, int fn, const float* x, const float* y, float* out, uint32_t n)
{
    if (!dev || !x || !y || !out) return fail(GMUPT_ERR_INVALID_ARGUMENT, "gmupt_debug_detmath: null argument");
    if (n == 0) return GMUPT_OK;
    HIP_TRY(hipSetDevice(dev->id));
    float *dx = nullptr, *dy = nullptr, *dout = nullptr;
    HIP_TRY(hipMalloc((void**)&dx, (size_t)n * 4)); HIP_TRY(hipMalloc((void**)&dy, (size_t)n * 4)); HIP_TRY(hipMalloc((void**)&dout, (size_t)n * 4));
    HIP_TRY(hipMemcpy(dx, x, (size_t)n * 4, hipMemcpyHostToDevice)); HIP_TRY(hipMemcpy(dy, y, (size_t)n * 4, hipMemcpyHostToDevice));
    launch_detmath(fn, dx, dy, dout, n, nullptr);
    HIP_TRY(hipGetLastError());
    HIP_TRY(hipMemcpy(out, dout, (size_t)n * 4, hipMemcpyDeviceToHost));
    (void)hipFree(dx); (void)hipFree(dy); (void)hipFree(dout);
    return GMUPT_OK;
}

static_assert(sizeof(gmupt_lbvh_info) == 48 && offsetof(gmupt_lbvh_info, ms) == 40, "gmupt_lbvh_info layout");

extern "C" void gmupt_lbvh_default_params(gmupt_lbvh_params* p) { if (p) p->max_leaf_size = 4; }

static void lbvh_fill_info(gmupt_lbvh_info* info, const LbResult& res, uint32_t numTris, double ms)
{
    if (!info) return;
    info->num_nodes = res.numNodes; info->num_leaves = res.numLeaves; info->depth = res.depth; info->num_tris = numTris;
    for (int k = 0; k < 3; k++) { info->root_min[k] = res.rootMin[k]; info->root_max[k] = res.rootMax[k]; }
    info->ms = ms;
}

static int lbvh_leaf_size(const char* fn, const gmupt_lbvh_params* params, uint32_t* L)
{
    *L = params ? params->max_leaf_size : 4u;
    if (*L < 1 || *L > kLbMaxLeaf) return fail(GMUPT_ERR_INVALID_ARGUMENT, "%s: max_leaf_size %u outside 1..%u", fn, *L, kLbMaxLeaf);
    return GMUPT_OK;
}

extern "C" int gmupt_lbvh_build_host(const float* verts, uint32_t num_verts, const int32_t* indices, uint32_t num_tris, const uint32_t* vertex_material,
                                     const gmupt_lbvh_params* params, gmupt_bvh_node* nodes_out, gmupt_triangle* tris_out, int32_t* ref_triangle_out,
                                     gmupt_lbvh_info* info)
{
    if (!verts || !indices || !nodes_out || !tris_out || num_verts == 0 || num_tris == 0) return fail(GMUPT_ERR_INVALID_ARGUMENT, "gmupt_lbvh_build_host: null or empty array");
    if (num_tris > kLbMaxTris) return fail(GMUPT_ERR_INVALID_ARGUMENT, "gmupt_lbvh_build_host: more than 2^30 triangles");
    uint32_t L;
    int rc = lbvh_leaf_size("gmupt_lbvh_build_host", params, &L);
    if (rc != GMUPT_OK) return rc;
    LbResult res{};
    int status = GMUPT_OK;
    const std::string err = lbvh_build_host(verts, num_verts, indices, num_tris, vertex_material, L, nodes_out, tris_out, ref_triangle_out, res, &status);
    if (status != GMUPT_OK) return fail(status, "gmupt_lbvh_build_host: %s", err.c_str());
    lbvh_fill_info(info, res, num_tris, 0.0);
    return GMUPT_OK;
}

struct gmupt_lbvh { gmupt_device* dev; hipStream_t stream = nullptr; hipEvent_t ev[2] = { nullptr, nullptr }; void* scratch = nullptr; uint32_t capTris = 0; size_t sortTemp = 0; };

extern "C" int gmupt_lbvh_create(gmupt_device* dev, gmupt_lbvh** out)
{
    if (!dev || !out) return fail(GMUPT_ERR_INVALID_ARGUMENT, "gmupt_lbvh_create: null argument");
    *out = nullptr;
    gmupt_lbvh* h = new (std::nothrow) gmupt_lbvh();
    if (!h) return fail(GMUPT_ERR_OUT_OF_MEMORY, "gmupt_lbvh_create: out of host memory");
    h->dev = dev;
    hipError_t e = hipSetDevice(dev->id);
    if (e == hipSuccess) e = hipStreamCreate(&h->stream);
    for (hipEvent_t& ev : h->ev) if (e == hipSuccess) e = hipEventCreate(&ev);
    if (e != hipSuccess) { gmupt_lbvh_destroy(h); return fail(GMUPT_ERR_HIP, "gmupt_lbvh_create: %s", hipGetErrorString(e)); }
    *out = h;
    return GMUPT_OK;
}

extern "C" void gmupt_lbvh_destroy(gmupt_lbvh* h)
{
    if (!h) return;
    (void)hipSetDevice(h->dev->id);
    if (h->stream) { (void)hipStreamSynchronize(h->stream); (void)hipStreamDestroy(h->stream); }
    for (hipEvent_t ev : h->ev) if (ev) (void)hipEventDestroy(ev);
    if (h->scratch) (void)hipFree(h->scratch);
    delete h;
}

static int lbvh_output_buffer(gmupt_device* dev, gmupt_buffer_kind kind, size_t elems, const void* src, hipStream_t s, gmupt_buffer** out)
{
    gmupt_buffer* b = new (std::nothrow) gmupt_buffer();
    if (!b) return fail(GMUPT_ERR_OUT_OF_MEMORY, "gmupt_lbvh_build: out of host memory");
    b->dev = dev; b->kind = kind; b->elems = elems; b->bytes = elems * kind_stride(kind); b->dptr = nullptr;
    hipError_t e = hipMalloc(&b->dptr, b->bytes + 16);
    if (e == hipSuccess) e = hipMemsetAsync((char*)b->dptr + b->bytes, 0, 16, s);
    if (e == hipSuccess) e = hipMemcpyAsync(b->dptr, src, b->bytes, hipMemcpyDeviceToDevice, s);
    if (e != hipSuccess) { if (b->dptr) (void)hipFree(b->dptr); delete b; return fail(GMUPT_ERR_HIP, "gmupt_lbvh_build(%zu bytes): %s", elems * kind_stride(kind), hipGetErrorString(e)); }
    *out = b;
    return GMUPT_OK;
}

extern "C" int gmupt_lbvh_build(gmupt_lbvh* h, const gmupt_buffer* vertices, const int32_t* device_indices, uint32_t num_tris, const uint32_t* device_vertex_material,
                                const gmupt_lbvh_params* params, gmupt_buffer** nodes_out, gmupt_buffer** triangles_out, int32_t* device_ref_triangle,
                                gmupt_lbvh_info* info)
{
    if (nodes_out) *nodes_out = nullptr;
    if (triangles_out) *triangles_out = nullptr;
    if (!h || !vertices || !device_indices || !nodes_out || !triangles_out) return fail(GMUPT_ERR_INVALID_ARGUMENT, "gmupt_lbvh_build: null argument");
    if (vertices->kind != GMUPT_BUFFER_VERTICES || vertices->dev != h->dev) return fail(GMUPT_ERR_INVALID_ARGUMENT, "gmupt_lbvh_build: not a vertex buffer of the builder's device");
    if (vertices->elems == 0 || num_tris == 0) return fail(GMUPT_ERR_INVALID_ARGUMENT, "gmupt_lbvh_build: empty mesh");
    if (num_tris > kLbMaxTris || vertices->elems > 0x7FFFFFFFu) return fail(GMUPT_ERR_INVALID_ARGUMENT, "gmupt_lbvh_build: more than 2^30 triangles or 2^31 - 1 vertices");
    if (((uintptr_t)device_indices | (uintptr_t)device_vertex_material | (uintptr_t)device_ref_triangle) & 3) return fail(GMUPT_ERR_INVALID_ARGUMENT, "gmupt_lbvh_build: misaligned pointer");
    uint32_t L;
    int rc = lbvh_leaf_size("gmupt_lbvh_build", params, &L);
    if (rc != GMUPT_OK) return rc;
    HIP_TRY(hipSetDevice(h->dev->id));
    size_t sortTemp = 0;
    HIP_TRY(lbvh_sort_temp_bytes(num_tris, &sortTemp));
// ... 97 lines not shown
```

gmu-path-tracer_amd/csrc/pt_device.hpp:

```cpp
#pragma once
#include <hip/hip_runtime.h>
#include <cstdint>
#include "../../include/gmupt.h"

namespace gmupt {

enum Field : uint32_t {
    F_RAY_OX, F_RAY_OY, F_RAY_OZ, F_RAY_DX, F_RAY_DY, F_RAY_DZ,
    F_MAT_R, F_MAT_G, F_MAT_B, F_MAT_METALLIC, F_MAT_ROUGHNESS,
    F_NRM_X, F_NRM_Y, F_NRM_Z,
    F_SP_X, F_SP_Y, F_SP_Z,
    F_BARY_X, F_BARY_Y, F_BARY_Z,
    F_HIT_DIST,
    F_TRI_0, F_TRI_1, F_TRI_2, F_TRI_MAT,
    F_SH_OX, F_SH_OY, F_SH_OZ, F_SH_DX, F_SH_DY, F_SH_DZ,
    F_LIGHT_IDX, F_LIGHT_DIST, F_IN_SHADOW,
    F_RAD_R, F_RAD_G, F_RAD_B,
    F_THR_R, F_THR_G, F_THR_B,
    F_LTHR_R, F_LTHR_G, F_LTHR_B,
    F_DL_R, F_DL_G, F_DL_B,
    F_PATH_LEN, F_SCR_X, F_SCR_Y, F_IS_EMITTER,
    F_COUNT
};
static_assert(F_COUNT == 50, "50 words per path");

enum SlotClass : uint8_t { CLS_UE4 = 0, CLS_GLASS = 1, CLS_ENDED = 2, CLS_RETIRED = 3, CLS_NONE = 4, CLS_MASK = 0x0F, CLS_SHADOW_BIT = 0x10 };
constexpr int kNumCounts = 4;
#ifndef GMUPT_SCAN_GROUP
#define GMUPT_SCAN_GROUP 64
#endif
constexpr uint32_t kScanGroup = GMUPT_SCAN_GROUP;

enum Counter : uint32_t { QC_NEWPATH = 0, QC_LASTPATHCNT = 1, QC_MATUE4 = 2, QC_MATGLASS = 3, QC_EXT_UE4_OFFSET = 4, QC_EXT_GLASS_OFFSET = 5, QC_SHADOWRAY = 6, QC_EXT_COUNT = 7 };
enum Queue : uint32_t { Q_NEWPATH = 0, Q_MAT_UE4 = 1, Q_MAT_GLASS = 2, Q_EXT_RAY = 3, Q_SHADOW_RAY = 4 };

constexpr uint32_t kQueueHole = 0xFFFFFFFFu;
constexpr uint32_t kListEnd = 0xFFFFFFFFu;
constexpr int kBlock = 256;

struct DevStats {
    unsigned long long pathsGenerated, pathsCompleted, segments;
    unsigned long long extRays, extInner, extLeaves, extTris;
    unsigned long long shRays, shInner, shLeaves, shTris;
    unsigned long long extWaveInner, extWaveTris, shWaveInner, shWaveTris;
    unsigned long long extDepthHist[32];
    unsigned long long laneCensus[4];
    unsigned long long castWaves, castWaveClocks, castWaveClocksMax;
    unsigned long long castDrainClocks, castDrainIters, castDrainBusyLanes;
    unsigned long long castWaveEndHist[32];
    unsigned long long rayInnerHist[32];
    unsigned long long extTopInner, shTopInner;
    unsigned long long castHelperSubtrees;
    unsigned long long castNestedHelpers;
    unsigned long long castRedoRays;
    unsigned long long widePairFetches;
    unsigned long long wideBoxTests;
    unsigned long long wideIters, wideGeneralIters;
    uint32_t activePaths;
    uint32_t stackOverflow;
};

struct alignas(16) DNode { float4 mn; float4 mx; int4 link; };
static_assert(sizeof(DNode) == sizeof(gmupt_bvh_node), "node layout");

struct SceneView {
    const DNode* nodes;
    const gmupt_triangle* tris;
    const float* verts;
    const gmupt_light* lights;
    const gmupt_tri_props* props;
    const gmupt_material* materials;
    uint32_t numNodes, numTris, numVerts, numMaterials;
    const uint8_t* tex[3];
    uint32_t texSize[3], texLayers[3];
};

struct alignas(64) Node64 { float a[4], b[4], c[4]; int32_t d[4]; };
struct alignas(16) Tri48 { float r0[4], r1[4], r2[4]; };
static_assert(sizeof(Node64) == 64 && sizeof(Tri48) == 48, "packed traversal records");

struct alignas(128) WNode { float p[6][4]; int32_t link[4]; int32_t aux[4]; };
static_assert(sizeof(WNode) == 128, "one wide node per 128-byte line");

struct alignas(16) TriPair { float w[20]; };
static_assert(sizeof(TriPair) == 80, "packed triangle pairs");

struct alignas(64) Rec64 { float q[16]; };

#ifndef GMUPT_TOP_NODES
#define GMUPT_TOP_NODES 768
#endif
#ifndef GMUPT_DEEP_TOP_NODES
#define GMUPT_DEEP_TOP_NODES 1280
#endif
constexpr int kDeepTopTreeNodes = GMUPT_DEEP_TOP_NODES;
constexpr int kTopTreeNodes = GMUPT_TOP_NODES;

struct TravScene {
    const Rec64* recs;
    uint32_t triBase;
    const Node64* nodes;
    const Tri48* tris;
    int32_t rootDesc;
    uint32_t topCount;
    uint32_t topCountDeep;
    uint32_t maxDepth;
    float rootMin[3], rootMax[3];
    const WNode* wnodes;
    uint32_t wideCount;
    uint32_t wideTopCount;
    uint32_t wideStackBound;
    int32_t wideRootDesc;
    const TriPair* pairs;
    const uint32_t* pairRef;
    uint32_t numPairs;
};

struct RenderParams {
    float* state;
    uint32_t P, L;
    uint8_t* cls;
    uint32_t* listNext;
    uint32_t* listHead;
    float* sample;
    uint32_t* blockCounts;
    uint32_t nBlocks;
    uint32_t* groupTotals;
    uint32_t nGroups;
    uint32_t groupParity;
    uint32_t* queues;
    uint32_t* qc;
    DevStats* stats;
    float4* fb;
    uint32_t fbW, fbH;
    uint32_t tileEnabled, tileX0, tileY0;
    uint32_t budget, maxDepth;
    int* ovfStack;
    uint32_t ovfStride;
    uint32_t raysPerWave;
    uint32_t* travCounters;
    uint32_t travGridBlocks;
    uint32_t extendPrune;
    uint32_t shadowPrune;
    uint32_t PS;
    uint32_t tuneRefill, tuneTriThresh;
    uint32_t tuneWideSteps;
    uint32_t wideQuarterTail;
    uint32_t xcdBins;
    uint32_t castLoopCap;
    gmupt_camera_buffer cam;
    SceneView scene;
    TravScene trav;
};

}
```

gmu-path-tracer_amd/csrc/pt_kernel_util.hpp:

```cpp
#pragma once
#include "pt_device.hpp"
#include "detmath.hpp"

namespace gmupt {

__device__ __forceinline__ float ldf(const RenderParams& p, uint32_t f, uint32_t i) { return p.state[(size_t)f * p.PS + i]; }
__device__ __forceinline__ uint32_t ldu(const RenderParams& p, uint32_t f, uint32_t i) { return __builtin_bit_cast(uint32_t, p.state[(size_t)f * p.PS + i]); }
__device__ __forceinline__ void stf(const RenderParams& p, uint32_t f, uint32_t i, float v) { p.state[(size_t)f * p.PS + i] = v; }
__device__ __forceinline__ void stu(const RenderParams& p, uint32_t f, uint32_t i, uint32_t v) { p.state[(size_t)f * p.PS + i] = __builtin_bit_cast(float, v); }
__device__ __forceinline__ f3 ld3(const RenderParams& p, uint32_t f, uint32_t i) { return mk3(ldf(p, f, i), ldf(p, f + 1, i), ldf(p, f + 2, i)); }
__device__ __forceinline__ void st3(const RenderParams& p, uint32_t f, uint32_t i, f3 v) { stf(p, f, i, v.x); stf(p, f + 1, i, v.y); stf(p, f + 2, i, v.z); }

__device__ __forceinline__ uint32_t lane_id() { return __builtin_amdgcn_mbcnt_hi(~0u, __builtin_amdgcn_mbcnt_lo(~0u, 0u)); }
__device__ __forceinline__ uint32_t prefix_rank(unsigned long long mask)
{
    return __builtin_amdgcn_mbcnt_hi((uint32_t)(mask >> 32), __builtin_amdgcn_mbcnt_lo((uint32_t)mask, 0u));
}

__device__ __forceinline__ uint32_t cam_width(const gmupt_camera_buffer& c) { return (uint32_t)(1.0f / c.pixelSize[0]); }
__device__ __forceinline__ uint32_t cam_height(const gmupt_camera_buffer& c) { return (uint32_t)(1.0f / c.pixelSize[1]); }

__device__ __forceinline__ uint32_t pixel_index(const RenderParams& p, uint32_t cx, uint32_t cy)
{
    uint32_t lx = cx - (p.tileEnabled ? p.tileX0 : 0u), ly = cy - (p.tileEnabled ? p.tileY0 : 0u);
    if (lx >= p.fbW || ly >= p.fbH) return kListEnd;
    return ly * p.fbW + lx;
}


}
```

gmu-path-tracer_amd/csrc/pt_kernels.hip:

```cpp
#include "pt_device.hpp"
#include "detmath.hpp"
#include "pt_kernel_util.hpp"
#include "pt_shading.hpp"

namespace gmupt {

__device__ __forceinline__ float schlickFresnel(float r0, float theta)
{
    float m = hsaturate(1.0f - theta);
    float m2 = m * m;
    return r0 - (1.0f - r0) * m2 * m2 * m;
}
__device__ __forceinline__ float GGXTrowbridgeReitz(float XdotY, float alpha)
{
    float a2 = alpha * alpha;
    float x = XdotY * XdotY * (a2 - 1.0f) + 1.0f;
    return a2 / (kPi * x * x);
}
__device__ __forceinline__ float smithSchlickGGX(float XdotY, float alpha)
{
    float a1 = alpha + 1.0f;
    float k = (a1 * a1) / 8.0f;
    return XdotY / (XdotY * (1.0f - k) + k);
}
__device__ __forceinline__ float lightFalloff(float distance, float radius)
{
    float q = distance / radius;
    float q2 = q * q;
    float n = hsaturate(1.0f - q2 * q2);
    return (n * n) / (distance * distance + 1.0f);
}
__device__ __forceinline__ float powerHeuristic(float rayPdf, float lightPdf)
{
    float t = rayPdf * rayPdf;
    return t / (lightPdf * lightPdf + t);
}

__device__ __forceinline__ void publish_block_counts(const RenderParams& p, int c)
{
    __shared__ uint32_t s_cnt[kNumCounts][kBlock / 64];
    const uint32_t wave = threadIdx.x >> 6;
    unsigned long long b0 = __ballot((c & CLS_MASK) == CLS_UE4), b1 = __ballot(c == CLS_GLASS), b2 = __ballot(c == CLS_ENDED), b3 = __ballot(c == (CLS_UE4 | CLS_SHADOW_BIT));
    if ((threadIdx.x & 63) == 0) { s_cnt[0][wave] = __popcll(b0); s_cnt[1][wave] = __popcll(b1); s_cnt[2][wave] = __popcll(b2); s_cnt[3][wave] = __popcll(b3); }
    __syncthreads();
    if (threadIdx.x < kNumCounts) {
        uint32_t s = 0;
        for (int w = 0; w < kBlock / 64; w++) s += s_cnt[threadIdx.x][w];
        p.blockCounts[threadIdx.x * p.nBlocks + blockIdx.x] = s;
        if (s) atomicAdd(&p.groupTotals[((size_t)p.groupParity * kNumCounts + threadIdx.x) * p.nGroups + blockIdx.x / kScanGroup], s);
    }
}

__global__ __launch_bounds__(kBlock) void k_clear(RenderParams p)
{
    const uint32_t i = blockIdx.x * kBlock + threadIdx.x;
    uint32_t w = p.tileEnabled ? p.fbW : cam_width(p.cam), h = p.tileEnabled ? p.fbH : cam_height(p.cam);
    uint32_t npix = w * h; if (npix > p.fbW * p.fbH) npix = p.fbW * p.fbH;
    for (uint32_t k = i; k < npix; k += gridDim.x * kBlock) { p.fb[k].w = __builtin_bit_cast(float, 0u); p.listHead[k] = kListEnd; }
    int c = CLS_NONE;
    if (i < p.L) { c = CLS_ENDED; p.cls[i] = CLS_ENDED; }
    publish_block_counts(p, c);
}

__global__ __launch_bounds__(kBlock) void k_logic(RenderParams p)
{
    const uint32_t i = blockIdx.x * kBlock + threadIdx.x;
    int c = CLS_NONE;
    if (i < p.L) {
        c = p.cls[i];
        if (c != CLS_RETIRED) {
            Rng g; g.seed(i, p.cam.randomSeed[0], p.cam.randomSeed[1]);
            bool pathEliminated = false;
            f3 throughput = ld3(p, F_THR_R, i);
            f3 radiance = ld3(p, F_RAD_R, i);
            const uint32_t isEmitter = ldu(p, F_IS_EMITTER, i);
            uint32_t pl = 0;
            if (isEmitter > 0) {
                const f3 e = sample_light_color(p.scene.lights, isEmitter);
                radiance = radiance + e * throughput;
                pathEliminated = true;
            } else {
                if (!ldu(p, F_IN_SHADOW, i)) radiance = radiance + ld3(p, F_DL_R, i) * throughput;
                throughput = throughput * ld3(p, F_LTHR_R, i);
                if (throughput.x <= 0.0f && throughput.y <= 0.0f && throughput.z <= 0.0f) pathEliminated = true;
                if (ldf(p, F_HIT_DIST, i) == kFltMax) {
                    radiance = radiance + throughput * mk3(p.cam.envColor[0], p.cam.envColor[1], p.cam.envColor[2]);
                    pathEliminated = true;
                }
                pl = ldu(p, F_PATH_LEN, i);
                if (pl > 200) {
                    float pr = hmax(throughput.x, hmax(throughput.y, throughput.z));
                    if (g.next() > pr * 0.004f) pathEliminated = true;
                    throughput = throughput * (1.0f / pr);
                }
                if (p.maxDepth && pl >= p.maxDepth) pathEliminated = true;
            }

            if (pathEliminated) {
                c = CLS_ENDED;
                f3 r = mk3(hsaturate(radiance.x), hsaturate(radiance.y), hsaturate(radiance.z));
                r = r / (r + mk3(1.0f, 1.0f, 1.0f));
                const float gm = 1.0f / 2.2f;
                r = mk3(dpow(r.x, gm), dpow(r.y, gm), dpow(r.z, gm));
                p.sample[i] = r.x; p.sample[(size_t)p.P + i] = r.y; p.sample[(size_t)2 * p.P + i] = r.z;
                const uint32_t pix = pixel_index(p, ldu(p, F_SCR_X, i), ldu(p, F_SCR_Y, i));
                uint32_t prev = kListEnd;
                if (pix != kListEnd) prev = atomicExch(&p.listHead[pix], i);
                p.listNext[i] = prev;
            } else {
                const HitProps hp = material_hit_properties(p.scene, ldu(p, F_TRI_0, i), ldu(p, F_TRI_1, i), ldu(p, F_TRI_2, i), ldu(p, F_TRI_MAT, i),
                                                            ld3(p, F_BARY_X, i), [&]() { return ld3(p, F_RAY_DX, i); });
                const f3 normal = hp.normal;
                st3(p, F_MAT_R, i, hp.color);
                stf(p, F_MAT_METALLIC, i, hp.metallic); stf(p, F_MAT_ROUGHNESS, i, hp.roughness);
                st3(p, F_NRM_X, i, normal);
                c = (hp.materialType == GMUPT_MATERIAL_UE4) ? CLS_UE4 : CLS_GLASS;

                uint32_t lightIndex = (uint32_t)(g.next() * (float)p.cam.lightCount);
                float z = 1.0f - 2.0f * g.next();
                float rr = dsqrt(hmax(0.0f, 1.0f - z * z));
                float phi = 2.0f * kPi * g.next();
                float x = rr * dcos(phi);
                float y = rr * dsin(phi);
                const gmupt_light L = p.scene.lights[lightIndex < GMUPT_MAX_LIGHTS ? lightIndex : GMUPT_MAX_LIGHTS - 1];
                f3 lightPosition = mk3(L.position[0], L.position[1], L.position[2]) + mk3(x, y, z) * L.radius;
                f3 surfacePos = ld3(p, F_SP_X, i) + normal * kEpsilonOffset;
                f3 lightDir = lightPosition - surfacePos;
                float distance = length3(lightDir);
                lightDir = normalize3(lightDir);
                stu(p, F_LIGHT_IDX, i, lightIndex);
                st3(p, F_SH_OX, i, surfacePos);
                st3(p, F_SH_DX, i, lightDir);
                stf(p, F_LIGHT_DIST, i, distance - kEpsilonOffset);
                if (c == CLS_UE4 && dot3(lightDir, normal) > 0.0f) c |= CLS_SHADOW_BIT;

                st3(p, F_RAD_R, i, radiance);
                st3(p, F_THR_R, i, throughput);
                stu(p, F_PATH_LEN, i, pl + 1u);
                stu(p, F_IN_SHADOW, i, 1u);
            }
            p.cls[i] = (uint8_t)c;
        }
    }
    publish_block_counts(p, c);
}

struct Ue4State { f3 rayDir; f3 baseColor; float metallic, roughness; f3 normal; };

__device__ __forceinline__ f3 ue4Sample(const Ue4State& st, Rng& g)
{
    const f3 N = st.normal;
    const f3 V = neg3(st.rayDir);
    const float r0 = g.next(), r1 = g.next();
    const float diffuseRatio = 1.0f - st.metallic;
    const f3 up = dabs(N.z) < 0.999f ? mk3(0.0f, 0.0f, 1.0f) : mk3(1.0f, 0.0f, 0.0f);
    const f3 tangent = normalize3(cross3(up, N));
    const f3 bitangent = cross3(N, tangent);
    f3 direction;
    if (g.next() < diffuseRatio) {
        float x = dsqrt(r0);
        float phi = 2.0f * kPi * r1;
        float dx = x * dcos(phi);
        float dy = x * dsin(phi);
        float dz = dsqrt(hmax(0.0f, 1.0f - dx * dx - dy * dy));
        direction = (tangent * dx + bitangent * dy) + N * dz;
    } else {
        float a = st.roughness * st.roughness;
        float phi = 2.0f * kPi * r0;
        float cosTheta = dsqrt((1.0f - r1) / (1.0f + (a * a - 1.0f) * r1));
        float sinTheta = dsqrt(1.0f - cosTheta * cosTheta);
        float hx = sinTheta * dcos(phi);
        float hy = sinTheta * dsin(phi);
        float hz = cosTheta;
        direction = (tangent * hx + bitangent * hy) + N * hz;
        direction = direction * (2.0f * dot3(V, direction)) - V;
    }
    return direction;
}

__device__ __forceinline__ float ue4Pdf(const Ue4State& st, f3 direction)
{
    const f3 N = st.normal, V = neg3(st.rayDir), L = direction;
    const float diffuseRatio = 1.0f - st.metallic;
    const float specularRatio = 1.0f - diffuseRatio;
    const f3 H = normalize3(L + V);
    const float NdotH = dabs(dot3(N, H));
    const float pdfGGXTR = GGXTrowbridgeReitz(NdotH, st.roughness * st.roughness) * NdotH;
    const float pdfSpec = pdfGGXTR / (4.0f * dabs(dot3(V, H)));
    const float pdfDiff = dabs(dot3(L, N)) * (1.0f / kPi);
    return diffuseRatio * pdfDiff + specularRatio * pdfSpec;
}

__device__ __forceinline__ f3 ue4Evaluate(const Ue4State& st, f3 direction)
{
    const f3 N = st.normal, V = neg3(st.rayDir), L = direction;
    const float NdotL = dot3(N, L), NdotV = dot3(N, V);
    if (NdotL <= 0.0f || NdotV <= 0.0f) return mk3(0.0f, 0.0f, 0.0f);
    const f3 H = normalize3(L + V);
    const float NdotH = dot3(N, H), LdotH = dot3(L, H);
    const float D = GGXTrowbridgeReitz(NdotH, st.roughness * st.roughness);
    const float G = smithSchlickGGX(NdotL, st.roughness) * smithSchlickGGX(NdotV, st.roughness);
    const f3 sc = mk3(0.037f + st.metallic * (st.baseColor.x - 0.037f),
                      0.037f + st.metallic * (st.baseColor.y - 0.037f),
                      0.037f + st.metallic * (st.baseColor.z - 0.037f));
    const float w = 1.0f - LdotH;
    const float w2 = w * w;
    const float fc = w2 * w2 * w;
    const f3 F = mk3((1.0f - fc) * sc.x + fc, (1.0f - fc) * sc.y + fc, (1.0f - fc) * sc.z + fc);
    const float den = 4.0f * NdotL * NdotV;
    const float om = 1.0f - st.metallic;
    return mk3((st.baseColor.x / kPi) * om + (D * F.x * G) / den,
               (st.baseColor.y / kPi) * om + (D * F.y * G) / den,
               (st.baseColor.z / kPi) * om + (D * F.z * G) / den);
}

__device__ __forceinline__ void stage_ue4(const RenderParams& p, uint32_t queueIndex, uint32_t index, uint32_t shadowRank, uint32_t extOffset)
{
    Rng g; g.seed(queueIndex, p.cam.randomSeed[0], p.cam.randomSeed[1]);
    Ue4State st;
    st.rayDir = ld3(p, F_RAY_DX, index);
    st.normal = ld3(p, F_NRM_X, index);
    st.baseColor = ld3(p, F_MAT_R, index);
    st.metallic = ldf(p, F_MAT_METALLIC, index);
    st.roughness = ldf(p, F_MAT_ROUGHNESS, index);

    const f3 bsdfDir = ue4Sample(st, g);
    const float pdf = ue4Pdf(st, bsdfDir);
    f3 throughput = mk3(0.0f, 0.0f, 0.0f);
    if (pdf > 0.0f) {
        const f3 e = ue4Evaluate(st, bsdfDir);
        const float an = dabs(dot3(st.normal, bsdfDir));
        throughput = mk3(e.x * an / pdf, e.y * an / pdf, e.z * an / pdf);
    }
    st3(p, F_LTHR_R, index, throughput);
    const f3 surfacePoint = ld3(p, F_SP_X, index);
    st3(p, F_RAY_OX, index, surfacePoint + bsdfDir * kEpsilonOffset);
    st3(p, F_RAY_DX, index, bsdfDir);
    p.queues[(size_t)Q_EXT_RAY * p.P + extOffset + queueIndex] = index;

    const f3 lightDir = ld3(p, F_SH_DX, index);
    if (dot3(lightDir, st.normal) > 0.0f) {
        const uint32_t lightIndex = ldu(p, F_LIGHT_IDX, index);
        const float distance = ldf(p, F_LIGHT_DIST, index);
        const gmupt_light L = p.scene.lights[lightIndex < GMUPT_MAX_LIGHTS ? lightIndex : GMUPT_MAX_LIGHTS - 1];
        const float lightPdf = distance * distance / (4.0f * kPi * L.radius * L.radius);
        const float bsdfPdf = ue4Pdf(st, lightDir);
        const float ph = powerHeuristic(lightPdf, bsdfPdf);
        const f3 e = ue4Evaluate(st, lightDir);
        const float lc = (float)p.cam.lightCount;
        const float fo = lightFalloff(distance, L.falloff);
        st3(p, F_DL_R, index, mk3(ph * e.x * L.emission[0] * lc * fo, ph * e.y * L.emission[1] * lc * fo, ph * e.z * L.emission[2] * lc * fo));
        const uint32_t pos = shadowRank;
        p.queues[(size_t)Q_SHADOW_RAY * p.P + pos] = index;
    }
}

__device__ __forceinline__ void stage_glass(const RenderParams& p, uint32_t queueIndex, uint32_t index, uint32_t extOffset)
{
    Rng g; g.seed(queueIndex, p.cam.randomSeed[0], p.cam.randomSeed[1]);
    const f3 rayDir = ld3(p, F_RAY_DX, index);
    const f3 stNormal = ld3(p, F_NRM_X, index);
    const f3 baseColor = ld3(p, F_MAT_R, index);

    const f3 normal = dot3(stNormal, rayDir) <= 0.0f ? stNormal : stNormal * -1.0f;
    const float n1 = 1.0f, n2 = 1.458f;
    float r0 = (n1 - n2) / (n1 + n2);
    r0 = r0 * r0;
    const float theta = dot3(neg3(rayDir), normal);
    const float probability = schlickFresnel(r0, theta);
    const float eta = dot3(stNormal, normal) > 0.0f ? (n1 / n2) : (n2 / n1);
    const float dn = dot3(normal, rayDir);
    const float k = 1.0f - eta * eta * (1.0f - dn * dn);
    f3 refr = mk3(0.0f, 0.0f, 0.0f);
    if (!(k < 0.0f)) refr = rayDir * eta - normal * (eta * dn + dsqrt(k));
    const f3 transDirection = normalize3(refr);
    const float cos2t = 1.0f - eta * eta * (1.0f - theta * theta);
    const float rnd = g.next();
    f3 bsdfDir = transDirection;
    if (cos2t < 0.0f || rnd < probability)
// ... 210 lines not shown
```

gmu-path-tracer_amd/csrc/pt_traverse_deferred.hpp:

```cpp
#pragma once
#include "pt_traverse_common.hpp"

namespace gmupt {

#ifndef GMUPT_DEF_STACK
#define GMUPT_DEF_STACK 24
#endif
#ifndef GMUPT_DEF_FIFO
#define GMUPT_DEF_FIFO 4
#endif
#ifndef GMUPT_DEF_BLOCK
#define GMUPT_DEF_BLOCK 1024
#endif
constexpr int kDefBlock = GMUPT_DEF_BLOCK;
constexpr int kDefStack = GMUPT_DEF_STACK;
constexpr int kFifo = GMUPT_DEF_FIFO;
static_assert((kDefStack + kFifo) * kDefBlock * 4 + kTopTreeNodes * 64 <= 160 * 1024, "LDS of one CU");
#ifndef GMUPT_DEEP_STACK
#define GMUPT_DEEP_STACK 16
#endif
constexpr int kDeepStack = GMUPT_DEEP_STACK;
template <bool OVF> constexpr int kDefLdsStack = OVF ? kDeepStack : kDefStack;
template <bool OVF> constexpr int kDefLdsTop = OVF ? kDeepTopTreeNodes : kTopTreeNodes;
template <bool OVF> __device__ __forceinline__ uint32_t top_count(const TravScene& ts) { return OVF ? ts.topCountDeep : ts.topCount; }
// ... 9 lines not shown
    {
        if (!OVF || ptr < kDefLdsStack<OVF>) lds[ptr * kDefBlock] = v;
        else if (ptr < kMaxStack + 1) ovf[(size_t)(ptr - kDefLdsStack<OVF>) * ovfStride] = v;
        else atomicOr(&st->stackOverflow, 1u);
        ptr++;
    }
    __device__ __forceinline__ int pop()
    {
        --ptr;
        if (!OVF || ptr < kDefLdsStack<OVF>) return lds[ptr * kDefBlock];
        if (ptr < kMaxStack + 1) return ovf[(size_t)(ptr - kDefLdsStack<OVF>) * ovfStride];
        return kDone;
    }
};

typedef float vec4f __attribute__((ext_vector_type(4)));
typedef int vec2i __attribute__((ext_vector_type(2)));
#define GMUPT_AS_LDS __attribute__((address_space(3)))
#define GMUPT_AS_GLOBAL __attribute__((address_space(1)))

template <bool TOP>
__device__ __forceinline__ void load_node(const TravScene& ts, const float4* s_top, uint32_t topCount, int cur, vec4f& a, vec4f& b, vec4f& c, vec2i& d)
{
    const bool inTop = TOP && (uint32_t)cur < topCount;
    if (inTop) {
        const GMUPT_AS_LDS vec4f* n = (const GMUPT_AS_LDS vec4f*)(s_top) + cur * 4;
        a = n[0]; b = n[1]; c = n[2]; d = *(const GMUPT_AS_LDS vec2i*)(n + 3);
    }
    asm volatile("" ::: "memory");
    if (!inTop) {
        const GMUPT_AS_GLOBAL vec4f* n = (const GMUPT_AS_GLOBAL vec4f*)(ts.nodes) + (size_t)cur * 4;
        a = n[0]; b = n[1]; c = n[2];
        const unsigned long long links = *(const GMUPT_AS_GLOBAL unsigned long long*)(n + 3);
        d.x = (int)(uint32_t)links; d.y = (int)(uint32_t)(links >> 32);
    }
}

typedef uint32_t vec4u __attribute__((ext_vector_type(4)));
typedef uint32_t vec2u __attribute__((ext_vector_type(2)));
constexpr int kBufferRsrcFlags = 0x00020000;

__device__ __forceinline__ __amdgpu_buffer_rsrc_t make_rsrc(const void* base, uint32_t bytes)
{
    return __builtin_amdgcn_make_buffer_rsrc(const_cast<void*>(base), 0, (int)bytes, kBufferRsrcFlags);
}

template <bool TOP>
__device__ __forceinline__ void load_node_buf(__amdgpu_buffer_rsrc_t nodes, const float4* s_top, uint32_t topCount, int cur, vec4f& a, vec4f& b, vec4f& c, vec2i& d)
{
    const bool inTop = TOP && (uint32_t)cur < topCount;
    if (inTop) {
        const GMUPT_AS_LDS vec4f* n = (const GMUPT_AS_LDS vec4f*)(s_top) + cur * 4;
        a = n[0]; b = n[1]; c = n[2]; d = *(const GMUPT_AS_LDS vec2i*)(n + 3);
    }
    asm volatile("" ::: "memory");
    if (!inTop) {
        const int off = cur * 64;
        a = __builtin_bit_cast(vec4f, __builtin_amdgcn_raw_buffer_load_b128(nodes, off, 0, 0));
        b = __builtin_bit_cast(vec4f, __builtin_amdgcn_raw_buffer_load_b128(nodes, off + 16, 0, 0));
        c = __builtin_bit_cast(vec4f, __builtin_amdgcn_raw_buffer_load_b128(nodes, off + 32, 0, 0));
        d = __builtin_bit_cast(vec2i, __builtin_amdgcn_raw_buffer_load_b64(nodes, off + 48, 0, 0));
    }
}

typedef float vec2f __attribute__((ext_vector_type(2)));
__device__ __forceinline__ void tri_fetch_buf(__amdgpu_buffer_rsrc_t tris, int i, vec4f& r0, vec4f& r1, vec2f& r2)
{
    const int off = i * 48;
    r0 = __builtin_bit_cast(vec4f, __builtin_amdgcn_raw_buffer_load_b128(tris, off, 0, 0));
    r1 = __builtin_bit_cast(vec4f, __builtin_amdgcn_raw_buffer_load_b128(tris, off + 16, 0, 0));
    r2 = __builtin_bit_cast(vec2f, __builtin_amdgcn_raw_buffer_load_b64(tris, off + 32, 0, 0));
}

template <bool OVF>
__device__ __forceinline__ int inner_compute(const vec4f a, const vec4f b, const vec4f c, const vec2i d, f3 o, f3 invdir, DefStack<OVF>& stk, DevStats* dst)
{
    const float leftHit = ray_box(a.x, a.y, a.z, a.w, b.x, b.y, o, invdir);
    const float rightHit = ray_box(b.z, b.w, c.x, c.y, c.z, c.w, o, invdir);
    const bool l = leftHit > 0.0f, r = rightHit > 0.0f;
    const bool swap = leftHit > rightHit;
    if (l && r) { stk.push(swap ? d.x : d.y, dst); return swap ? d.y : d.x; }
    if (l | r) return l ? d.x : d.y;
    return stk.pop();
}

template <bool OVF>
__device__ __forceinline__ int inner_compute_flat(const vec4f a, const vec4f b, const vec4f c, const vec2i d, f3 o, f3 invdir, DefStack<OVF>& stk, DevStats* dst)
{
    const float leftHit = ray_box(a.x, a.y, a.z, a.w, b.x, b.y, o, invdir);
    const float rightHit = ray_box(b.z, b.w, c.x, c.y, c.z, c.w, o, invdir);
    const bool l = leftHit > 0.0f, r = rightHit > 0.0f;
    const bool swap = leftHit > rightHit;
    const bool both = l && r;
    const int nearChild = (both && swap) || (!l) ? d.y : d.x;
    const int farChild = swap ? d.x : d.y;
    if (both) stk.push(farChild, dst);
    int next = nearChild;
    if (!(l | r)) next = stk.pop();
    return next;
}

template <bool OVF, bool TOP>
__device__ __forceinline__ int inner_step_d(const TravScene& ts, const float4* s_top, int cur, f3 o, f3 invdir, DefStack<OVF>& stk, DevStats* dst)
{
    vec4f a, b, c; vec2i d;
    load_node<TOP>(ts, s_top, top_count<OVF>(ts), cur, a, b, c, d);
    return inner_compute<OVF>(a, b, c, d, o, invdir, stk, dst);
}

template <bool OVF, bool TOP>
__device__ __forceinline__ int inner_step_pruned(const TravScene& ts, const float4* s_top, int cur, f3 o, f3 invdir, float limitT, DefStack<OVF>& stk, DevStats* dst)
{
    vec4f a, b, c; vec2i d;
    load_node<TOP>(ts, s_top, top_count<OVF>(ts), cur, a, b, c, d);
    float le, re;
    const float leftHit = ray_box_entry(a.x, a.y, a.z, a.w, b.x, b.y, o, invdir, le);
    const float rightHit = ray_box_entry(b.z, b.w, c.x, c.y, c.z, c.w, o, invdir, re);
    const bool l = leftHit > 0.0f && le <= limitT, r = rightHit > 0.0f && re <= limitT;
    const bool swap = leftHit > rightHit;
    if (l && r) { stk.push(swap ? d.x : d.y, dst); return swap ? d.y : d.x; }
    if (l | r) return l ? d.x : d.y;
    return stk.pop();
}

#define GMUPT_DEF_LDS(TOP) \
    __shared__ int s_stack[kDefLdsStack<OVF> * kDefBlock]; \
    __shared__ int s_fifo[kFifo * kDefBlock]; \
    __shared__ float4 s_top[TOP ? kDefLdsTop<OVF> * 4 : 4]; \
    if (TOP) { \
        const float4* src = reinterpret_cast<const float4*>(p.trav.nodes); \
        for (uint32_t k = threadIdx.x; k < top_count<OVF>(p.trav) * 4u; k += kDefBlock) s_top[k] = src[k]; \
        __syncthreads(); \
    }

#define GMUPT_LIGHT_SPHERES(LIGHTS, COUNT, O, D, DIST, INDEX) \
    uint32_t INDEX = 0; \
    { const uint32_t lc = (COUNT) < GMUPT_MAX_LIGHTS ? (COUNT) : GMUPT_MAX_LIGHTS; \
      for (uint32_t li = 0; li < lc; li++) { \
          const gmupt_light L = (LIGHTS)[li]; \
          const f3 position = mk3(L.position[0], L.position[1], L.position[2]) - (O); \
          const float radius2 = L.radius * L.radius; \
          const float tca = dot3(position, (D)); \
          const float d2 = dot3(position, position) - tca * tca; \
          if (d2 > radius2) continue; \
          const float thc = dsqrt(radius2 - d2); \
          float t0 = tca - thc; \
          const float t1 = tca + thc; \
          if (t0 < 0.0f) t0 = t1; \
          if (t0 > 0.0f && t0 < (DIST)) { (DIST) = t0; INDEX = li + 1; } \
      } }

__device__ __forceinline__ void finish_extension_ray(const RenderParams& p, uint32_t index, f3 o, f3 d, float distance, float hu, float hv, int hitRef)
{
    if (distance < kFltMax) {
        st3(p, F_SP_X, index, o + d * distance);
        st3(p, F_BARY_X, index, mk3(1.0f - hu - hv, hu, hv));
        const int4 T = *reinterpret_cast<const int4*>(&p.scene.tris[hitRef]);
        stu(p, F_TRI_0, index, (uint32_t)T.x); stu(p, F_TRI_1, index, (uint32_t)T.y);
        stu(p, F_TRI_2, index, (uint32_t)T.z); stu(p, F_TRI_MAT, index, (uint32_t)T.w);
    }
    GMUPT_LIGHT_SPHERES(p.scene.lights, p.cam.lightCount, o, d, distance, lightIndex)
    stu(p, F_IS_EMITTER, index, lightIndex);
    stf(p, F_HIT_DIST, index, distance);
}

__device__ __forceinline__ void shadow_counter_epilogue(const RenderParams& p)
{
    if (blockIdx.x == 0 && threadIdx.x == 0) {
        const uint32_t q0 = p.qc[QC_NEWPATH], q1 = p.qc[QC_LASTPATHCNT];
        p.qc[QC_NEWPATH] = 0; p.qc[QC_LASTPATHCNT] = q0 + q1; p.qc[QC_MATUE4] = 0; p.qc[QC_MATGLASS] = 0;
    }
}

#define GMUPT_DEF_LAUNCH(KERNEL, TOP, REPS, BURST) \
    do { if (ovf) { if (stats) hipLaunchKernelGGL((KERNEL<true, true, TOP, REPS, BURST>), dim3(pb), dim3(kDefBlock), 0, s, p); \
                    else hipLaunchKernelGGL((KERNEL<false, true, TOP, REPS, BURST>), dim3(pb), dim3(kDefBlock), 0, s, p); } \
         else { if (stats) hipLaunchKernelGGL((KERNEL<true, false, TOP, REPS, BURST>), dim3(pb), dim3(kDefBlock), 0, s, p); \
                else hipLaunchKernelGGL((KERNEL<false, false, TOP, REPS, BURST>), dim3(pb), dim3(kDefBlock), 0, s, p); } } while (0)

}
```

include/gmupt.h:

```cpp
#ifndef GMUPT_H
#define GMUPT_H

#include <stddef.h>
#include <stdint.h>

#ifdef __cplusplus
extern "C" {
#endif

#define GMUPT_MAX_LIGHTS 128
#define GMUPT_PATHCOUNT (1u << 21)
#define GMUPT_REF_GRID_THREADS (34u * 8u * 256u)
#define GMUPT_STATE_BYTES 248u

typedef enum {
    GMUPT_OK = 0,
    GMUPT_ERR_INVALID_ARGUMENT = -1,
    GMUPT_ERR_HIP = -2,
    GMUPT_ERR_OUT_OF_MEMORY = -3,
    GMUPT_ERR_NOT_BOUND = -4,
    GMUPT_ERR_UNSUPPORTED = -5,
    GMUPT_ERR_IO = -6,
    GMUPT_ERR_CAST_FAULT = -7
} gmupt_status;
// ... 68 lines not shown
#define GMUPT_STAT_STACK_OVERFLOW 1u
#define GMUPT_STAT_FUSED_CAST 2u
#define GMUPT_STAT_CAST_FETCH 4u
#define GMUPT_STAT_CAST_ABORTED 16u
#define GMUPT_STAT_CAST_WIDE 32u
#define GMUPT_STAT_STACK_SPILL 8u
typedef struct {
    uint64_t iterations;
    uint64_t paths_generated;
    uint64_t paths_completed;
    uint64_t segments;
    uint32_t active_paths;
    uint32_t flags;
    uint64_t ext_rays, ext_inner, ext_leaves, ext_tris;
    uint64_t sh_rays, sh_inner, sh_leaves, sh_tris;
    double ms_logic, ms_scan, ms_accumulate, ms_material, ms_extend, ms_shadow;
    uint64_t timed_iterations;
    uint64_t ext_wave_inner, ext_wave_tris, sh_wave_inner, sh_wave_tris;
    uint64_t ext_depth_hist[32];
    uint64_t lane_census[4];
    uint64_t cast_waves, cast_wave_ticks, cast_wave_ticks_max;
    uint64_t cast_drain_ticks, cast_drain_iters, cast_drain_busy_lanes;
    uint64_t cast_wave_end_hist[32];
    uint64_t ray_inner_hist[32];
    uint64_t ext_top_inner, sh_top_inner;
    uint64_t cast_helper_subtrees;
    uint64_t cast_nested_helpers;
    uint64_t cast_redo_rays;
    uint64_t wide_nodes, wide_top_nodes, wide_stack_bound;
    uint64_t wide_pairs, wide_pair_fetches;
    uint64_t wide_box_tests;
    uint64_t wide_iterations, wide_general_iterations;
} gmupt_stats;
int gmupt_get_stats(gmupt_renderer* r, gmupt_stats* out);
int gmupt_reset_stats(gmupt_renderer* r);
int gmupt_enable_timing(gmupt_renderer* r, int mode);

typedef struct gmupt_camera gmupt_camera;
int gmupt_render_budget(gmupt_renderer* r, gmupt_camera* camera, uint32_t max_iterations, uint32_t* iters);

typedef struct { float origin[3]; float tmax; float direction[3]; uint32_t pad; } gmupt_ray;
typedef struct {
    float t, u, v;
    int32_t triangle;
    uint32_t light;
    uint32_t material;
    uint32_t pad[2];
} gmupt_hit;
typedef struct {
    uint32_t flags;
    uint32_t pad_;
    uint64_t redo_rays;
    double ms;
} gmupt_trace_info;
int gmupt_trace_rays(gmupt_renderer* r, const gmupt_ray* closest, uint32_t n_closest, gmupt_hit* hits,
                     const gmupt_ray* any, uint32_t n_any, uint32_t* occluded, uint32_t light_count, gmupt_trace_info* info );
int gmupt_camera_pick_ray(const gmupt_camera_buffer* cam, float px, float py, gmupt_ray* out);
int gmupt_pick(gmupt_renderer* r, float px, float py, uint32_t light_count, gmupt_ray* ray_out, gmupt_hit* hit_out);

typedef struct {
    float albedo[3];   float depth;
    float normal[3];   float roughness;
    float position[3]; float metallic;
    int32_t triangle; uint32_t material; uint32_t light; uint32_t coverage;
} gmupt_aov;
#define GMUPT_AOV_MAX_SAMPLES 8
#define GMUPT_AOV_CHUNK_RAYS (1u << 21)
int gmupt_render_aovs(gmupt_renderer* r, uint32_t samples, gmupt_aov* out, size_t bytes, gmupt_trace_info* info );
int gmupt_aov_ray(const gmupt_camera_buffer* cam, uint32_t x, uint32_t y, uint32_t samples, uint32_t k, gmupt_ray* out);

typedef struct {
    uint32_t passes;
    float sigma_color;
    float sigma_normal;
    float sigma_plane;
    float sigma_albedo;
} gmupt_denoise_params;
#define GMUPT_DENOISE_MAX_PASSES 5
void gmupt_denoise_default_params(gmupt_denoise_params* p);
int gmupt_denoise_image(gmupt_renderer* r, const float* beauty_rgba, const gmupt_aov* aov, uint32_t width, uint32_t height,
                        const gmupt_denoise_params* p, float* out_rgba, size_t out_bytes, float* ms );
int gmupt_render_denoised(gmupt_renderer* r, uint32_t aov_samples, const gmupt_denoise_params* p, float* out_rgba, size_t bytes,
                          gmupt_trace_info* info );
int gmupt_denoise_host(const float* beauty_rgba, const gmupt_aov* aov, uint32_t width, uint32_t height, const gmupt_denoise_params* p,
                       float* out_rgba, size_t out_bytes, uint32_t threads);

typedef struct {
    float color[3];    float count;
    float normal[3];   uint32_t material;
    float position[3]; uint32_t valid;
} gmupt_history;
typedef struct {
    gmupt_denoise_params spatial;
    float history_cap;
    float min_normal_cos;
    float plane_dist;
} gmupt_temporal_params;
#define GMUPT_TEMPORAL_MAX_CAP 65536.0f
void gmupt_temporal_default_params(gmupt_temporal_params* p);
typedef struct gmupt_temporal gmupt_temporal;
int gmupt_temporal_create(gmupt_renderer* r, gmupt_temporal** out);
void gmupt_temporal_destroy(gmupt_temporal* t);
int gmupt_temporal_reset(gmupt_temporal* t);
int gmupt_temporal_denoise_image(gmupt_temporal* t, const float* beauty_rgba, const gmupt_aov* aov, const gmupt_camera_buffer* cam,
                                 uint32_t x0, uint32_t y0, uint32_t width, uint32_t height, int new_accumulation,
                                 const gmupt_temporal_params* p, float* out_rgba, size_t out_bytes, float* ms );
int gmupt_render_denoised_temporal(gmupt_renderer* r, gmupt_temporal* t, uint32_t aov_samples, const gmupt_temporal_params* p,
                                   float* out_rgba, size_t bytes, gmupt_trace_info* info );
int gmupt_temporal_integrate_host(const float* beauty_rgba, const gmupt_aov* aov, uint32_t width, uint32_t height,
                                  const gmupt_history* prev, const gmupt_camera_buffer* prev_cam, uint32_t prev_x0, uint32_t prev_y0,
                                  uint32_t prev_width, uint32_t prev_height, const gmupt_temporal_params* p,
                                  float* out_rgba, gmupt_history* out_history, uint32_t threads);

#define GMUPT_REFIT_FLAT_CHILD 1u
#define GMUPT_REFIT_VARIANTS_BUILD 2u
typedef struct { uint32_t rebuilt; uint32_t reason; uint32_t levels; uint32_t opened_nodes; double ms; } gmupt_refit_info;
int gmupt_bvh_refit_host(gmupt_bvh_node* nodes, uint32_t num_nodes, const gmupt_triangle* tris, uint32_t num_tris,
                         const float* verts, uint32_t num_verts, uint32_t threads);
int gmupt_renderer_refit(gmupt_renderer* r, gmupt_refit_info* info );

typedef struct { float prev_position[3]; uint32_t flags; } gmupt_motion;
int gmupt_render_aovs_motion(gmupt_renderer* r, uint32_t samples, const float* prev_verts, uint32_t num_verts, gmupt_aov* aov_out, size_t aov_bytes,
                             gmupt_motion* motion_out, size_t motion_bytes, gmupt_trace_info* info );
int gmupt_motion_host(const gmupt_hit* hits, const gmupt_aov* aov, size_t n, const gmupt_triangle* tris, uint32_t num_tris,
                      const float* verts_now, const float* verts_prev, uint32_t num_verts, gmupt_motion* out);
int gmupt_temporal_integrate_motion_host(const float* beauty_rgba, const gmupt_aov* aov, const gmupt_motion* motion ,
                                         uint32_t width, uint32_t height,
                                         const gmupt_history* prev, const gmupt_camera_buffer* prev_cam, uint32_t prev_x0, uint32_t prev_y0,
                                         uint32_t prev_width, uint32_t prev_height, const gmupt_temporal_params* p,
                                         float* out_rgba, gmupt_history* out_history, uint32_t threads);
int gmupt_temporal_denoise_image_motion(gmupt_temporal* t, const float* beauty_rgba, const gmupt_aov* aov, const gmupt_motion* motion ,
                                        const gmupt_camera_buffer* cam, uint32_t x0, uint32_t y0, uint32_t width, uint32_t height,
                                        int new_accumulation, const gmupt_temporal_params* p, float* out_rgba, size_t out_bytes,
                                        float* ms );
int gmupt_render_denoised_temporal_motion(gmupt_renderer* r, gmupt_temporal* t, uint32_t aov_samples, const gmupt_temporal_params* p,
                                          float* out_rgba, size_t bytes, gmupt_trace_info* info );

typedef struct { uint32_t max_leaf_size; } gmupt_lbvh_params;
void gmupt_lbvh_default_params(gmupt_lbvh_params* p);
typedef struct { uint32_t num_nodes, num_leaves, depth, num_tris; float root_min[3], root_max[3]; double ms; } gmupt_lbvh_info;
int gmupt_lbvh_build_host(const float* verts, uint32_t num_verts, const int32_t* indices, uint32_t num_tris, const uint32_t* vertex_material ,
                          const gmupt_lbvh_params* params , gmupt_bvh_node* nodes_out, gmupt_triangle* tris_out,
                          int32_t* ref_triangle_out , gmupt_lbvh_info* info );
typedef struct gmupt_lbvh gmupt_lbvh;
int gmupt_lbvh_create(gmupt_device* dev, gmupt_lbvh** out);
void gmupt_lbvh_destroy(gmupt_lbvh* h);
int gmupt_lbvh_build(gmupt_lbvh* h, const gmupt_buffer* vertices, const int32_t* device_indices, uint32_t num_tris,
                     const uint32_t* device_vertex_material , const gmupt_lbvh_params* params ,
                     gmupt_buffer** nodes_out, gmupt_buffer** triangles_out, int32_t* device_ref_triangle ,
                     gmupt_lbvh_info* info );

int gmupt_debug_read_path_state(gmupt_renderer* r, void* dst, size_t bytes);
int gmupt_debug_write_path_state(gmupt_renderer* r, const void* src, size_t bytes);
int gmupt_debug_read_queues(gmupt_renderer* r, uint32_t* dst, size_t bytes);
int gmupt_debug_write_queues(gmupt_renderer* r, const uint32_t* src, size_t bytes);
int gmupt_debug_write_counters(gmupt_renderer* r, const uint32_t in[8]);
int gmupt_debug_write_framebuffer(gmupt_renderer* r, const float* rgba, size_t bytes);
typedef enum { GMUPT_STAGE_SHADE = 0 , GMUPT_STAGE_EXTEND = 1, GMUPT_STAGE_SHADOW = 2,
               GMUPT_STAGE_RAYCASTS = 3  } gmupt_stage;
int gmupt_debug_run_stage(gmupt_renderer* r, gmupt_stage stage);
int gmupt_debug_detmath(gmupt_device* dev, int fn, const float* x, const float* y, float* out, uint32_t n);

typedef struct gmupt_travtables gmupt_travtables;
typedef enum { GMUPT_TT_NODE64 = 0, GMUPT_TT_TRI48 = 1, GMUPT_TT_TRIPAIR = 2, GMUPT_TT_PAIRREF = 3, GMUPT_TT_WNODE = 4, GMUPT_TT_REC64 = 5,
               GMUPT_TT_SCALARS = 6, GMUPT_TT_LEVEL_NODES = 7, GMUPT_TT_LEVEL_OFF = 8, GMUPT_TT_NODE_MAP = 9, GMUPT_TT_WIDE_MAP = 10,
               GMUPT_TT_OPENED = 11 } gmupt_travtable_kind;
int gmupt_debug_travtables_build(const gmupt_bvh_node* nodes, uint32_t num_nodes, const gmupt_triangle* tris, uint32_t num_tris,
                                 const float* verts, uint32_t num_verts, int want_wide, int top_order_bfs, int node_pairing, gmupt_travtables** out);
const void* gmupt_debug_travtables_data(const gmupt_travtables* h, int which , size_t* bytes);
void gmupt_debug_travtables_destroy(gmupt_travtables* h);
int gmupt_debug_wide_tables_addressable(uint32_t wide_nodes, uint32_t num_tris, uint32_t num_pairs);

typedef struct {
    float split_alpha;
    int32_t max_depth;
    int32_t max_spatial_depth;
    int32_t min_leaf_size;
    int32_t max_leaf_size;
    float node_cost, tri_cost;
} gmupt_sbvh_params;
void gmupt_sbvh_default_params(gmupt_sbvh_params* p);
typedef struct gmupt_sbvh gmupt_sbvh;
int gmupt_sbvh_build(const float* vertices, uint32_t num_vertices, const int32_t* indices, uint32_t num_triangles,
                     const gmupt_sbvh_params* params, gmupt_sbvh** out);
uint32_t gmupt_sbvh_num_nodes(const gmupt_sbvh* h);
uint32_t gmupt_sbvh_num_references(const gmupt_sbvh* h);
float gmupt_sbvh_sah(const gmupt_sbvh* h);
uint32_t gmupt_sbvh_depth(const gmupt_sbvh* h);
int gmupt_sbvh_flatten(const gmupt_sbvh* h, const uint32_t* vertex_material, gmupt_bvh_node* nodes, gmupt_triangle* triangles, int32_t* ref_triangle);
void gmupt_sbvh_destroy(gmupt_sbvh* h);

int gmupt_camera_create(uint32_t width, uint32_t height, gmupt_camera** out);
void gmupt_camera_destroy(gmupt_camera* c);
void gmupt_camera_update_resolution(gmupt_camera* c, uint32_t width, uint32_t height);
void gmupt_camera_set_pose(gmupt_camera* c, float x, float y, float z, float pitch, float yaw);
void gmupt_camera_update(gmupt_camera* c, float dt);
void gmupt_camera_reset_accumulation(gmupt_camera* c);
void gmupt_camera_set_input(gmupt_camera* c, float mouse_dx, float mouse_dy, uint32_t keys_wsad);
gmupt_camera_buffer* gmupt_camera_get_buffer(gmupt_camera* c);

const char* gmupt_version(void);

#ifdef __cplusplus
}
#endif
#endif
```

Measured before the change: 15.33 Mpaths/s.

## Move per-path hit data into a 48-byte AoS hit record with vector stores

Splits twelve hit-related fields (surface point, hit distance, barycentrics, emitter index, triangle indices and material) out of the SoA path state into a per-path 48-byte record. The extension kernel writes it with three 16-byte stores, and the shade kernel reads it with three 16-byte loads instead of twelve scattered strided loads. The goal is fewer memory transactions and fewer touched cache lines per path. The cost is uncoalesced AoS access across lanes, which may waste bandwidth when neighbouring lanes handle non-adjacent paths, plus extra host pack/unpack code for debug state I/O.

```diff
diff --git a/gmu-path-tracer_amd/build.py b/gmu-path-tracer_amd/build.py
--- a/gmu-path-tracer_amd/build.py
+++ b/gmu-path-tracer_amd/build.py
@@ -6,8 +6,8 @@
 LIB = os.path.join(HERE, "libgmupt.so")
 
 DEVICE_SOURCES = ["csrc/pt_kernels.hip", "csrc/pt_traverse.hip", "csrc/pt_traverse_wide.hip", "csrc/pt_traverse_variants.hip", "csrc/pt_aov.hip", "csrc/pt_denoise.hip", "csrc/pt_temporal.hip", "csrc/pt_refit.hip", "csrc/pt_motion.hip", "csrc/pt_lbvh.hip", "csrc/gmupt_capi.hip"]
-HOST_SOURCES = ["csrc/pt_travtables.cpp", "csrc/pt_lbvh.cpp", "host/sbvh_builder.cpp", "host/Camera.cpp", "host/TextureLoader.cpp", "host/AvirResize.cpp"]
-HEADERS = ["csrc/pt_traverse_common.hpp", "csrc/pt_shading.hpp", "csrc/pt_denoise.hpp", "csrc/pt_temporal.hpp", "csrc/pt_refit.hpp", "csrc/pt_travtables.hpp", "csrc/pt_motion.hpp", "csrc/pt_lbvh.hpp", "csrc/pt_traverse_deferred.hpp", "csrc/pt_kernel_util.hpp", "host/MeshData.hpp", "host/BVHWrapper.hpp", "csrc/pt_device.hpp", "csrc/detmath.hpp", "host/sbvh_builder.hpp", "host/Camera.hpp", "host/TextureLoader.hpp", "host/png_reader.hpp", "host/Constants.hpp", "../include/gmupt.h"]
+HOST_SOURCES = ["csrc/pt_travtables.cpp", "csrc/pt_state_layout.cpp", "csrc/pt_lbvh.cpp", "host/sbvh_builder.cpp", "host/Camera.cpp", "host/TextureLoader.cpp", "host/AvirResize.cpp"]
+HEADERS = ["csrc/pt_traverse_common.hpp", "csrc/pt_shading.hpp", "csrc/pt_denoise.hpp", "csrc/pt_temporal.hpp", "csrc/pt_refit.hpp", "csrc/pt_travtables.hpp", "csrc/pt_motion.hpp", "csrc/pt_lbvh.hpp", "csrc/pt_traverse_deferred.hpp", "csrc/pt_kernel_util.hpp", "csrc/pt_state_layout.hpp", "host/MeshData.hpp", "host/BVHWrapper.hpp", "csrc/pt_device.hpp", "csrc/detmath.hpp", "host/sbvh_builder.hpp", "host/Camera.hpp", "host/TextureLoader.hpp", "host/png_reader.hpp", "host/Constants.hpp", "../include/gmupt.h"]
 
 FLAGS = [
     "--offload-arch=gfx950", "-O3", "-std=c++17", "-fPIC", "-shared",
diff --git a/gmu-path-tracer_amd/capi.py b/gmu-path-tracer_amd/capi.py
--- a/gmu-path-tracer_amd/capi.py
+++ b/gmu-path-tracer_amd/capi.py
@@ -218,6 +218,10 @@
     "gmupt_lbvh_build": (C.c_int, [_P, _P, _P, C.c_uint32, _P, C.POINTER(LbvhParams), C.POINTER(_P), C.POINTER(_P), _P, C.POINTER(LbvhInfo)]),
     "gmupt_debug_read_path_state": (C.c_int, [_P, _P, C.c_size_t]),
     "gmupt_debug_write_path_state": (C.c_int, [_P, _P, C.c_size_t]),
+    "gmupt_debug_read_hit_records": (C.c_int, [_P, _P, C.c_size_t]),
+    "gmupt_debug_write_hit_records": (C.c_int, [_P, _P, C.c_size_t]),
+    "gmupt_debug_path_state_pack": (C.c_int, [_P, C.c_size_t, C.c_size_t, _P, _P]),
+    "gmupt_debug_path_state_unpack": (C.c_int, [_P, _P, C.c_size_t, C.c_size_t, _P]),
     "gmupt_debug_read_queues": (C.c_int, [_P, _P, C.c_size_t]),
     "gmupt_debug_write_queues": (C.c_int, [_P, _P, C.c_size_t]),
     "gmupt_debug_write_counters": (C.c_int, [_P, C.POINTER(C.c_uint32 * 8)]),
@@ -380,6 +384,27 @@
     return out
 
 
+HITREC_WORDS = 12
+STATE_SOA_FIELDS = 38
+
+
+def path_state_pack(ref, pool, stride):
+    ref = np.ascontiguousarray(ref, dtype=np.uint8)
+    assert ref.nbytes == pool * STATE_BYTES and stride >= pool
+    state = np.full((STATE_SOA_FIELDS, stride), 0xA5A5A5A5, dtype=np.uint32)
+    rec = np.full((pool, HITREC_WORDS), 0xA5A5A5A5, dtype=np.uint32)
+    _check(lib().gmupt_debug_path_state_pack(_ptr(ref), pool, stride, _ptr(state), _ptr(rec)))
+    return state, rec
+
+
+def path_state_unpack(state, rec, pool, stride):
+    state = np.ascontiguousarray(state, dtype=np.uint32); rec = np.ascontiguousarray(rec, dtype=np.uint32)
+    assert state.size == STATE_SOA_FIELDS * stride and rec.size == pool * HITREC_WORDS
+    out = np.full(pool * STATE_BYTES, 0xA5, dtype=np.uint8)
+    _check(lib().gmupt_debug_path_state_unpack(_ptr(state), _ptr(rec), pool, stride, _ptr(out)))
+    return out
+
+
 def resize_square(rgba, new_size):
     rgba = np.ascontiguousarray(rgba, dtype=np.uint8)
     assert rgba.ndim == 3 and rgba.shape[0] == rgba.shape[1] and rgba.shape[2] == 4
@@ -632,6 +657,15 @@
     def write_path_state(self, raw):
         raw = np.ascontiguousarray(raw, dtype=np.uint8)
         _check(lib().gmupt_debug_write_path_state(self.h, _ptr(raw), raw.nbytes))
+
+    def read_hit_records(self):
+        out = np.empty(self.pool * HITREC_WORDS, dtype=np.uint32)
+        _check(lib().gmupt_debug_read_hit_records(self.h, _ptr(out), out.nbytes))
+        return out.reshape(self.pool, HITREC_WORDS)
+
+    def write_hit_records(self, rec):
+        rec = np.ascontiguousarray(rec, dtype=np.uint32)
+        _check(lib().gmupt_debug_write_hit_records(self.h, _ptr(rec), rec.nbytes))
 
     def read_queues(self):
         out = np.empty(self.pool * 5, dtype=np.uint32)
diff --git a/gmu-path-tracer_amd/csrc/gmupt_capi.hip b/gmu-path-tracer_amd/csrc/gmupt_capi.hip
--- a/gmu-path-tracer_amd/csrc/gmupt_capi.hip
+++ b/gmu-path-tracer_amd/csrc/gmupt_capi.hip
@@ -343,7 +343,7 @@
     if (r->desc.pool_paths == 0) r->desc.pool_paths = GMUPT_PATHCOUNT;
     if (r->desc.live_paths == 0 || r->desc.live_paths > r->desc.pool_paths) r->desc.live_paths = r->desc.pool_paths;
     const uint32_t P = r->desc.pool_paths, L = r->desc.live_paths;
-    if ((uint64_t)P * F_COUNT * 4ull > (200ull << 30)) { delete r; return fail(GMUPT_ERR_INVALID_ARGUMENT, "gmupt_renderer_create: pool of %u paths is too large", P); }
+    if ((uint64_t)P * (kSoaFields + kHitRecWords) * 4ull > (200ull << 30)) { delete r; return fail(GMUPT_ERR_INVALID_ARGUMENT, "gmupt_renderer_create: pool of %u paths is too large", P); }
 
     hipError_t e = hipSetDevice(dev->id);
     if (e == hipSuccess) e = hipStreamCreateWithFlags(&r->stream, hipStreamNonBlocking);
@@ -369,7 +369,8 @@
 
     int rc = GMUPT_OK;
     { const char* pad = std::getenv("GMUPT_STATE_PAD"); p.PS = P + (pad ? (uint32_t)std::atoi(pad) & ~63u : 1088u); }
-    if (rc == GMUPT_OK) rc = dev_alloc(r, (void**)&p.state, (size_t)F_COUNT * p.PS * 4, 0);
+    if (rc == GMUPT_OK) rc = dev_alloc(r, (void**)&p.state, state_words(p.PS) * 4, 0);
+    if (rc == GMUPT_OK) rc = dev_alloc(r, (void**)&p.hitrec, hitrec_words(P) * 4, 0);
     if (rc == GMUPT_OK) rc = dev_alloc(r, (void**)&p.cls, (size_t)P, CLS_ENDED);
     if (rc == GMUPT_OK) rc = dev_alloc(r, (void**)&p.listNext, (size_t)P * 4, 0xFF);
     if (rc == GMUPT_OK) rc = dev_alloc(r, (void**)&p.sample, (size_t)P * 12, 0);
@@ -1459,13 +1460,14 @@
 }
 
 namespace {
-struct FieldMap { uint32_t refOffset, slotBytes, comps, first; };
-const FieldMap kFieldMap[] = {
-    { 0, 16, 3, F_RAY_OX }, { 16, 16, 3, F_RAY_DX }, { 32, 16, 3, F_MAT_R }, { 48, 8, 2, F_MAT_METALLIC }, { 56, 16, 3, F_NRM_X },
-    { 72, 16, 3, F_SP_X }, { 88, 16, 3, F_BARY_X }, { 104, 4, 1, F_HIT_DIST }, { 108, 16, 4, F_TRI_0 }, { 124, 16, 3, F_SH_OX },
-    { 140, 16, 3, F_SH_DX }, { 156, 4, 1, F_LIGHT_IDX }, { 160, 4, 1, F_LIGHT_DIST }, { 164, 4, 1, F_IN_SHADOW }, { 168, 16, 3, F_RAD_R },
-    { 184, 16, 3, F_THR_R }, { 200, 16, 3, F_LTHR_R }, { 216, 16, 3, F_DL_R }, { 232, 4, 1, F_PATH_LEN }, { 236, 8, 2, F_SCR_X }, { 244, 4, 1, F_IS_EMITTER },
-};
+int download_path_state(gmupt_renderer* r, std::vector<uint32_t>& soa, std::vector<uint32_t>& rec)
+{
+    soa.resize(state_words(r->p.PS)); rec.resize(hitrec_words(r->p.P));
+    HIP_TRY(hipMemcpyAsync(soa.data(), r->p.state, soa.size() * 4, hipMemcpyDeviceToHost, r->stream));
+    HIP_TRY(hipMemcpyAsync(rec.data(), r->p.hitrec, rec.size() * 4, hipMemcpyDeviceToHost, r->stream));
+    HIP_TRY(hipStreamSynchronize(r->stream));
+    return GMUPT_OK;
+}
 }
 
 extern "C" int gmupt_debug_read_path_state(gmupt_renderer* r, void* dst, size_t bytes)
@@ -1474,17 +1476,10 @@
     const size_t P = r->p.P;
     if (bytes < P * GMUPT_STATE_BYTES) return fail(GMUPT_ERR_INVALID_ARGUMENT, "gmupt_debug_read_path_state: %zu bytes given, %zu needed", bytes, P * (size_t)GMUPT_STATE_BYTES);
     HIP_TRY(hipSetDevice(r->dev->id));
-    const size_t PS = r->p.PS;
-    std::vector<uint32_t> soa((size_t)F_COUNT * PS);
-    HIP_TRY(hipMemcpyAsync(soa.data(), r->p.state, soa.size() * 4, hipMemcpyDeviceToHost, r->stream));
-    HIP_TRY(hipStreamSynchronize(r->stream));
-    std::memset(dst, 0, P * GMUPT_STATE_BYTES);
-    uint8_t* out = (uint8_t*)dst;
-    for (const FieldMap& f : kFieldMap)
-        for (size_t i = 0; i < P; i++) {
-            uint32_t* o = (uint32_t*)(out + (size_t)f.refOffset * P + (size_t)f.slotBytes * i);
-            for (uint32_t c = 0; c < f.comps; c++) o[c] = soa[(size_t)(f.first + c) * PS + i];
-        }
+    std::vector<uint32_t> soa, rec;
+    const int rc = download_path_state(r, soa, rec);
+    if (rc != GMUPT_OK) return rc;
+    path_state_unpack(soa.data(), rec.data(), P, r->p.PS, dst);
     return GMUPT_OK;
 }
 
@@ -1494,16 +1489,47 @@
     const size_t P = r->p.P;
     if (bytes < P * GMUPT_STATE_BYTES) return fail(GMUPT_ERR_INVALID_ARGUMENT, "gmupt_debug_write_path_state: %zu bytes given, %zu needed", bytes, P * (size_t)GMUPT_STATE_BYTES);
     HIP_TRY(hipSetDevice(r->dev->id));
-    const size_t PS = r->p.PS;
-    std::vector<uint32_t> soa((size_t)F_COUNT * PS);
-    const uint8_t* in = (const uint8_t*)src;
-    for (const FieldMap& f : kFieldMap)
-        for (size_t i = 0; i < P; i++) {
-            const uint32_t* o = (const uint32_t*)(in + (size_t)f.refOffset * P + (size_t)f.slotBytes * i);
-            for (uint32_t c = 0; c < f.comps; c++) soa[(size_t)(f.first + c) * PS + i] = o[c];
-        }
+    std::vector<uint32_t> soa(state_words(r->p.PS)), rec(hitrec_words(P));
+    path_state_pack(src, P, r->p.PS, soa.data(), rec.data());
     HIP_TRY(hipMemcpyAsync(r->p.state, soa.data(), soa.size() * 4, hipMemcpyHostToDevice, r->stream));
-    HIP_TRY(hipStreamSynchronize(r->stream));
+    HIP_TRY(hipMemcpyAsync(r->p.hitrec, rec.data(), rec.size() * 4, hipMemcpyHostToDevice, r->stream));
+    HIP_TRY(hipStreamSynchronize(r->stream));
+    return GMUPT_OK;
+}
+
+extern "C" int gmupt_debug_read_hit_records(gmupt_renderer* r, uint32_t* dst, size_t bytes)
+{
+    if (!r || !dst) return fail(GMUPT_ERR_INVALID_ARGUMENT, "gmupt_debug_read_hit_records: null argument");
+    const size_t need = hitrec_words(r->p.P) * 4;
+    if (bytes < need) return fail(GMUPT_ERR_INVALID_ARGUMENT, "gmupt_debug_read_hit_records: %zu bytes given, %zu needed", bytes, need);
+    HIP_TRY(hipSetDevice(r->dev->id));
+    HIP_TRY(hipMemcpyAsync(dst, r->p.hitrec, need, hipMemcpyDeviceToHost, r->stream));
+    HIP_TRY(hipStreamSynchronize(r->stream));
+    return GMUPT_OK;
+}
+
+extern "C" int gmupt_debug_write_hit_records(gmupt_renderer* r, const uint32_t* src, size_t bytes)
+{
+    if (!r || !src) return fail(GMUPT_ERR_INVALID_ARGUMENT, "gmupt_debug_write_hit_records: null argument");
+    const size_t need = hitrec_words(r->p.P) * 4;
+    if (bytes < need) return fail(GMUPT_ERR_INVALID_ARGUMENT, "gmupt_debug_write_hit_records: %zu bytes given, %zu needed", bytes, need);
+    HIP_TRY(hipSetDevice(r->dev->id));
+    HIP_TRY(hipMemcpyAsync(r->p.hitrec, src, need, hipMemcpyHostToDevice, r->stream));
+    HIP_TRY(hipStreamSynchronize(r->stream));
+    return GMUPT_OK;
+}
+
+extern "C" int gmupt_debug_path_state_pack(const void* ref, size_t P, size_t stride, uint32_t* state, uint32_t* hitrec)
+{
+    if (!ref || !state || !hitrec || stride < P) return fail(GMUPT_ERR_INVALID_ARGUMENT, "gmupt_debug_path_state_pack: null argument or stride < P");
+    path_state_pack(ref, P, stride, state, hitrec);
+    return GMUPT_OK;
+}
+
+extern "C" int gmupt_debug_path_state_unpack(const uint32_t* state, const uint32_t* hitrec, size_t P, size_t stride, void* ref)
+{
+    if (!ref || !state || !hitrec || stride < P) return fail(GMUPT_ERR_INVALID_ARGUMENT, "gmupt_debug_path_state_unpack: null argument or stride < P");
+    path_state_unpack(state, hitrec, P, stride, ref);
     return GMUPT_OK;
 }
 
diff --git a/gmu-path-tracer_amd/csrc/pt_device.hpp b/gmu-path-tracer_amd/csrc/pt_device.hpp
--- a/gmu-path-tracer_amd/csrc/pt_device.hpp
+++ b/gmu-path-tracer_amd/csrc/pt_device.hpp
@@ -2,27 +2,9 @@
 #include <hip/hip_runtime.h>
 #include <cstdint>
 #include "../../include/gmupt.h"
+#include "pt_state_layout.hpp"
 
 namespace gmupt {
-
-enum Field : uint32_t {
-    F_RAY_OX, F_RAY_OY, F_RAY_OZ, F_RAY_DX, F_RAY_DY, F_RAY_DZ,
-    F_MAT_R, F_MAT_G, F_MAT_B, F_MAT_METALLIC, F_MAT_ROUGHNESS,
-    F_NRM_X, F_NRM_Y, F_NRM_Z,
-    F_SP_X, F_SP_Y, F_SP_Z,
-    F_BARY_X, F_BARY_Y, F_BARY_Z,
-    F_HIT_DIST,
-    F_TRI_0, F_TRI_1, F_TRI_2, F_TRI_MAT,
-    F_SH_OX, F_SH_OY, F_SH_OZ, F_SH_DX, F_SH_DY, F_SH_DZ,
-    F_LIGHT_IDX, F_LIGHT_DIST, F_IN_SHADOW,
-    F_RAD_R, F_RAD_G, F_RAD_B,
-    F_THR_R, F_THR_G, F_THR_B,
-    F_LTHR_R, F_LTHR_G, F_LTHR_B,
-    F_DL_R, F_DL_G, F_DL_B,
-    F_PATH_LEN, F_SCR_X, F_SCR_Y, F_IS_EMITTER,
-    F_COUNT
-};
-static_assert(F_COUNT == 50, "50 words per path");
 
 enum SlotClass : uint8_t { CLS_UE4 = 0, CLS_GLASS = 1, CLS_ENDED = 2, CLS_RETIRED = 3, CLS_NONE = 4, CLS_MASK = 0x0F, CLS_SHADOW_BIT = 0x10 };
 constexpr int kNumCounts = 4;
@@ -118,6 +100,7 @@
 
 struct RenderParams {
     float* state;
+    float* hitrec;
     uint32_t P, L;
     uint8_t* cls;
     uint32_t* listNext;
diff --git a/gmu-path-tracer_amd/csrc/pt_kernel_util.hpp b/gmu-path-tracer_amd/csrc/pt_kernel_util.hpp
--- a/gmu-path-tracer_amd/csrc/pt_kernel_util.hpp
+++ b/gmu-path-tracer_amd/csrc/pt_kernel_util.hpp
@@ -4,12 +4,18 @@
 
 namespace gmupt {
 
-__device__ __forceinline__ float ldf(const RenderParams& p, uint32_t f, uint32_t i) { return p.state[(size_t)f * p.PS + i]; }
-__device__ __forceinline__ uint32_t ldu(const RenderParams& p, uint32_t f, uint32_t i) { return __builtin_bit_cast(uint32_t, p.state[(size_t)f * p.PS + i]); }
-__device__ __forceinline__ void stf(const RenderParams& p, uint32_t f, uint32_t i, float v) { p.state[(size_t)f * p.PS + i] = v; }
-__device__ __forceinline__ void stu(const RenderParams& p, uint32_t f, uint32_t i, uint32_t v) { p.state[(size_t)f * p.PS + i] = __builtin_bit_cast(float, v); }
+__device__ __forceinline__ float* field_ptr(const RenderParams& p, uint32_t f, uint32_t i)
+{
+    return is_hitrec_field(f) ? p.hitrec + ((size_t)i * kHitRecWords + hitrec_word(f)) : p.state + ((size_t)soa_index(f) * p.PS + i);
+}
+__device__ __forceinline__ float ldf(const RenderParams& p, uint32_t f, uint32_t i) { return *field_ptr(p, f, i); }
+__device__ __forceinline__ uint32_t ldu(const RenderParams& p, uint32_t f, uint32_t i) { return __builtin_bit_cast(uint32_t, *field_ptr(p, f, i)); }
+__device__ __forceinline__ void stf(const RenderParams& p, uint32_t f, uint32_t i, float v) { *field_ptr(p, f, i) = v; }
+__device__ __forceinline__ void stu(const RenderParams& p, uint32_t f, uint32_t i, uint32_t v) { *field_ptr(p, f, i) = __builtin_bit_cast(float, v); }
 __device__ __forceinline__ f3 ld3(const RenderParams& p, uint32_t f, uint32_t i) { return mk3(ldf(p, f, i), ldf(p, f + 1, i), ldf(p, f + 2, i)); }
 __device__ __forceinline__ void st3(const RenderParams& p, uint32_t f, uint32_t i, f3 v) { stf(p, f, i, v.x); stf(p, f + 1, i, v.y); stf(p, f + 2, i, v.z); }
+
+__device__ __forceinline__ float4* hitrec_quarter(const RenderParams& p, uint32_t i, uint32_t q) { return reinterpret_cast<float4*>(p.hitrec + (size_t)i * kHitRecWords) + q; }
 
 __device__ __forceinline__ uint32_t lane_id() { return __builtin_amdgcn_mbcnt_hi(~0u, __builtin_amdgcn_mbcnt_lo(~0u, 0u)); }
 __device__ __forceinline__ uint32_t prefix_rank(unsigned long long mask)
diff --git a/gmu-path-tracer_amd/csrc/pt_kernels.hip b/gmu-path-tracer_amd/csrc/pt_kernels.hip
--- a/gmu-path-tracer_amd/csrc/pt_kernels.hip
+++ b/gmu-path-tracer_amd/csrc/pt_kernels.hip
@@ -71,9 +71,10 @@
         if (c != CLS_RETIRED) {
             Rng g; g.seed(i, p.cam.randomSeed[0], p.cam.randomSeed[1]);
             bool pathEliminated = false;
+            const float4 hitA = *hitrec_quarter(p, i, 0), hitB = *hitrec_quarter(p, i, 1), hitC = *hitrec_quarter(p, i, 2);
             f3 throughput = ld3(p, F_THR_R, i);
             f3 radiance = ld3(p, F_RAD_R, i);
-            const uint32_t isEmitter = ldu(p, F_IS_EMITTER, i);
+            const uint32_t isEmitter = __float_as_uint(hitB.w);
             uint32_t pl = 0;
             if (isEmitter > 0) {
                 const f3 e = sample_light_color(p.scene.lights, isEmitter);
@@ -83,7 +84,7 @@
                 if (!ldu(p, F_IN_SHADOW, i)) radiance = radiance + ld3(p, F_DL_R, i) * throughput;
                 throughput = throughput * ld3(p, F_LTHR_R, i);
                 if (throughput.x <= 0.0f && throughput.y <= 0.0f && throughput.z <= 0.0f) pathEliminated = true;
-                if (ldf(p, F_HIT_DIST, i) == kFltMax) {
+                if (hitA.w == kFltMax) {
                     radiance = radiance + throughput * mk3(p.cam.envColor[0], p.cam.envColor[1], p.cam.envColor[2]);
                     pathEliminated = true;
                 }
@@ -108,8 +109,8 @@
                 if (pix != kListEnd) prev = atomicExch(&p.listHead[pix], i);
                 p.listNext[i] = prev;
             } else {
-                const HitProps hp = material_hit_properties(p.scene, ldu(p, F_TRI_0, i), ldu(p, F_TRI_1, i), ldu(p, F_TRI_2, i), ldu(p, F_TRI_MAT, i),
-                                                            ld3(p, F_BARY_X, i), [&]() { return ld3(p, F_RAY_DX, i); });
+                const HitProps hp = material_hit_properties(p.scene, __float_as_uint(hitC.x), __float_as_uint(hitC.y), __float_as_uint(hitC.z), __float_as_uint(hitC.w),
+                                                            mk3(hitB.x, hitB.y, hitB.z), [&]() { return ld3(p, F_RAY_DX, i); });
                 const f3 normal = hp.normal;
                 st3(p, F_MAT_R, i, hp.color);
                 stf(p, F_MAT_METALLIC, i, hp.metallic); stf(p, F_MAT_ROUGHNESS, i, hp.roughness);
@@ -124,7 +125,7 @@
                 float y = rr * dsin(phi);
                 const gmupt_light L = p.scene.lights[lightIndex < GMUPT_MAX_LIGHTS ? lightIndex : GMUPT_MAX_LIGHTS - 1];
                 f3 lightPosition = mk3(L.position[0], L.position[1], L.position[2]) + mk3(x, y, z) * L.radius;
-                f3 surfacePos = ld3(p, F_SP_X, i) + normal * kEpsilonOffset;
+                f3 surfacePos = mk3(hitA.x, hitA.y, hitA.z) + normal * kEpsilonOffset;
                 f3 lightDir = lightPosition - surfacePos;
                 float distance = length3(lightDir);
                 lightDir = normalize3(lightDir);
diff --git a/gmu-path-tracer_amd/csrc/pt_state_layout.cpp b/gmu-path-tracer_amd/csrc/pt_state_layout.cpp
--- /dev/null
+++ b/gmu-path-tracer_amd/csrc/pt_state_layout.cpp
@@ -0,0 +1,51 @@
+#include "pt_state_layout.hpp"
+#include <cstring>
+
+namespace gmupt {
+
+namespace {
+constexpr size_t kRefStateBytes = 248;
+struct FieldMap { uint32_t refOffset, slotBytes, comps, first; };
+const FieldMap kFieldMap[] = {
+    { 0, 16, 3, F_RAY_OX }, { 16, 16, 3, F_RAY_DX }, { 32, 16, 3, F_MAT_R }, { 48, 8, 2, F_MAT_METALLIC }, { 56, 16, 3, F_NRM_X },
+    { 72, 16, 3, F_SP_X }, { 88, 16, 3, F_BARY_X }, { 104, 4, 1, F_HIT_DIST }, { 108, 16, 4, F_TRI_0 }, { 124, 16, 3, F_SH_OX },
+    { 140, 16, 3, F_SH_DX }, { 156, 4, 1, F_LIGHT_IDX }, { 160, 4, 1, F_LIGHT_DIST }, { 164, 4, 1, F_IN_SHADOW }, { 168, 16, 3, F_RAD_R },
+    { 184, 16, 3, F_THR_R }, { 200, 16, 3, F_LTHR_R }, { 216, 16, 3, F_DL_R }, { 232, 4, 1, F_PATH_LEN }, { 236, 8, 2, F_SCR_X }, { 244, 4, 1, F_IS_EMITTER },
+};
+inline size_t word_index(uint32_t f, size_t i, size_t PS, bool& inRecord)
+{
+    inRecord = is_hitrec_field(f);
+    return inRecord ? i * kHitRecWords + hitrec_word(f) : (size_t)soa_index(f) * PS + i;
+}
+}
+
+void path_state_pack(const void* ref, size_t P, size_t PS, uint32_t* state, uint32_t* hitrec)
+{
+    std::memset(state, 0, state_words(PS) * 4);
+    std::memset(hitrec, 0, hitrec_words(P) * 4);
+    const uint8_t* in = (const uint8_t*)ref;
+    for (const FieldMap& f : kFieldMap)
+        for (size_t i = 0; i < P; i++) {
+            const uint8_t* o = in + (size_t)f.refOffset * P + (size_t)f.slotBytes * i;
+            for (uint32_t c = 0; c < f.comps; c++) {
+                bool rec; const size_t w = word_index(f.first + c, i, PS, rec);
+                std::memcpy((rec ? hitrec : state) + w, o + 4 * c, 4);
+            }
+        }
+}
+
+void path_state_unpack(const uint32_t* state, const uint32_t* hitrec, size_t P, size_t PS, void* ref)
+{
+    std::memset(ref, 0, P * kRefStateBytes);
+    uint8_t* out = (uint8_t*)ref;
+    for (const FieldMap& f : kFieldMap)
+        for (size_t i = 0; i < P; i++) {
+            uint8_t* o = out + (size_t)f.refOffset * P + (size_t)f.slotBytes * i;
+            for (uint32_t c = 0; c < f.comps; c++) {
+                bool rec; const size_t w = word_index(f.first + c, i, PS, rec);
+                std::memcpy(o + 4 * c, (rec ? hitrec : state) + w, 4);
+            }
+        }
+}
+
+}
diff --git a/gmu-path-tracer_amd/csrc/pt_state_layout.hpp b/gmu-path-tracer_amd/csrc/pt_state_layout.hpp
--- /dev/null
+++ b/gmu-path-tracer_amd/csrc/pt_state_layout.hpp
@@ -0,0 +1,46 @@
+#pragma once
+#include <cstddef>
+#include <cstdint>
+
+namespace gmupt {
+
+enum Field : uint32_t {
+    F_RAY_OX, F_RAY_OY, F_RAY_OZ, F_RAY_DX, F_RAY_DY, F_RAY_DZ,
+    F_MAT_R, F_MAT_G, F_MAT_B, F_MAT_METALLIC, F_MAT_ROUGHNESS,
+    F_NRM_X, F_NRM_Y, F_NRM_Z,
+    F_SP_X, F_SP_Y, F_SP_Z,
+    F_BARY_X, F_BARY_Y, F_BARY_Z,
+    F_HIT_DIST,
+    F_TRI_0, F_TRI_1, F_TRI_2, F_TRI_MAT,
+    F_SH_OX, F_SH_OY, F_SH_OZ, F_SH_DX, F_SH_DY, F_SH_DZ,
+    F_LIGHT_IDX, F_LIGHT_DIST, F_IN_SHADOW,
+    F_RAD_R, F_RAD_G, F_RAD_B,
+    F_THR_R, F_THR_G, F_THR_B,
+    F_LTHR_R, F_LTHR_G, F_LTHR_B,
+    F_DL_R, F_DL_G, F_DL_B,
+    F_PATH_LEN, F_SCR_X, F_SCR_Y, F_IS_EMITTER,
+    F_COUNT
+};
+static_assert(F_COUNT == 50, "50 words per path");
+
+constexpr uint32_t kHitRecWords = 12;
+constexpr uint32_t kHitRecFields = 12;
+constexpr uint32_t kSoaFields = F_COUNT - kHitRecFields;
+
+constexpr bool is_hitrec_field(uint32_t f) { return (f >= F_SP_X && f <= F_TRI_MAT) || f == F_IS_EMITTER; }
+constexpr uint32_t hitrec_word(uint32_t f)
+{
+    return f <= F_SP_Z ? f - F_SP_X : f <= F_BARY_Z ? 4u + (f - F_BARY_X) : f == F_HIT_DIST ? 3u : f == F_IS_EMITTER ? 7u : 8u + (f - F_TRI_0);
+}
+constexpr uint32_t soa_index(uint32_t f) { return f < F_SP_X ? f : f - (F_TRI_MAT + 1 - F_SP_X); }
+static_assert(kHitRecWords % 4 == 0, "a record is whole 16-byte stores");
+static_assert(F_TRI_MAT + 1 - F_SP_X == kHitRecFields - 1 && soa_index(F_SH_OX) == F_SP_X && soa_index(F_SCR_Y) == kSoaFields - 1, "the record fields are F_SP_X..F_TRI_MAT and F_IS_EMITTER");
+static_assert(hitrec_word(F_SP_Z) == 2 && hitrec_word(F_HIT_DIST) == 3 && hitrec_word(F_BARY_X) == 4 && hitrec_word(F_IS_EMITTER) == 7 && hitrec_word(F_TRI_0) == 8 && hitrec_word(F_TRI_MAT) == 11, "record order");
+
+constexpr size_t state_words(size_t PS) { return (size_t)kSoaFields * PS; }
+constexpr size_t hitrec_words(size_t P) { return (size_t)kHitRecWords * P; }
+
+void path_state_pack(const void* ref, size_t P, size_t PS, uint32_t* state, uint32_t* hitrec);
+void path_state_unpack(const uint32_t* state, const uint32_t* hitrec, size_t P, size_t PS, void* ref);
+
+}
diff --git a/gmu-path-tracer_amd/csrc/pt_traverse_deferred.hpp b/gmu-path-tracer_amd/csrc/pt_traverse_deferred.hpp
--- a/gmu-path-tracer_amd/csrc/pt_traverse_deferred.hpp
+++ b/gmu-path-tracer_amd/csrc/pt_traverse_deferred.hpp
@@ -185,16 +185,18 @@
 
 __device__ __forceinline__ void finish_extension_ray(const RenderParams& p, uint32_t index, f3 o, f3 d, float distance, float hu, float hv, int hitRef)
 {
-    if (distance < kFltMax) {
-        st3(p, F_SP_X, index, o + d * distance);
-        st3(p, F_BARY_X, index, mk3(1.0f - hu - hv, hu, hv));
-        const int4 T = *reinterpret_cast<const int4*>(&p.scene.tris[hitRef]);
-        stu(p, F_TRI_0, index, (uint32_t)T.x); stu(p, F_TRI_1, index, (uint32_t)T.y);
-        stu(p, F_TRI_2, index, (uint32_t)T.z); stu(p, F_TRI_MAT, index, (uint32_t)T.w);
-    }
+    const float triT = distance;
+    const bool triHit = triT < kFltMax;
+    if (triHit) *hitrec_quarter(p, index, 2) = *reinterpret_cast<const float4*>(&p.scene.tris[hitRef]);
     GMUPT_LIGHT_SPHERES(p.scene.lights, p.cam.lightCount, o, d, distance, lightIndex)
-    stu(p, F_IS_EMITTER, index, lightIndex);
-    stf(p, F_HIT_DIST, index, distance);
+    if (triHit) {
+        const f3 sp = o + d * triT, bary = mk3(1.0f - hu - hv, hu, hv);
+        *hitrec_quarter(p, index, 0) = make_float4(sp.x, sp.y, sp.z, distance);
+        *hitrec_quarter(p, index, 1) = make_float4(bary.x, bary.y, bary.z, __builtin_bit_cast(float, lightIndex));
+    } else {
+        stu(p, F_IS_EMITTER, index, lightIndex);
+        stf(p, F_HIT_DIST, index, distance);
+    }
 }
 
 __device__ __forceinline__ void shadow_counter_epilogue(const RenderParams& p)
diff --git a/include/gmupt.h b/include/gmupt.h
--- a/include/gmupt.h
+++ b/include/gmupt.h
@@ -244,6 +244,10 @@
 
 int gmupt_debug_read_path_state(gmupt_renderer* r, void* dst, size_t bytes);
 int gmupt_debug_write_path_state(gmupt_renderer* r, const void* src, size_t bytes);
+int gmupt_debug_read_hit_records(gmupt_renderer* r, uint32_t* dst, size_t bytes);
+int gmupt_debug_write_hit_records(gmupt_renderer* r, const uint32_t* src, size_t bytes);
+int gmupt_debug_path_state_pack(const void* ref, size_t P, size_t stride, uint32_t* state, uint32_t* hitrec);
+int gmupt_debug_path_state_unpack(const uint32_t* state, const uint32_t* hitrec, size_t P, size_t stride, void* ref);
 int gmupt_debug_read_queues(gmupt_renderer* r, uint32_t* dst, size_t bytes);
 int gmupt_debug_write_queues(gmupt_renderer* r, const uint32_t* src, size_t bytes);
 int gmupt_debug_write_counters(gmupt_renderer* r, const uint32_t in[8]);
```

New measurement: 15.41 Mpaths/s, median of 6. Within noise of the previous version (+0.5%).
